# zertovitch/zip-ada

Hardware: NVIDIA B200
Metric: bzip2_encode_MBps_900k (higher is better)
Workload: dtype u8

## Files before the change

zip-ada_b200/csrc/b2_api.cu:

```cuda
#include "b2_common.cuh"
#include "b2_kernels.h"
#include "../../include/b2gpu.h"

#include <algorithm>
#include <atomic>
#include <cmath>
#include <condition_variable>
#include <cstdlib>
#include <cstring>
#include <deque>
#include <chrono>
#include <map>
#include <mutex>
#include <string>
#include <thread>
#include <vector>
#include <unordered_set>

static thread_local std::string g_last_error = "";
void b2_set_error(const char *file, int line, const char *msg) {
  char buf[512];
  snprintf(buf, sizeof buf, "%s:%d: %s", file, line, msg);
  g_last_error = buf;
}
#define B2_FAIL(code, msg) do { b2_set_error(__FILE__, __LINE__, msg); return code; } while (0)
#define B2_TRY(x) do { int rc_ = (x); if (rc_) return rc_; } while (0)

namespace {

template <class T> struct DevBuf {
  T *p = nullptr; size_t cap = 0;
  int ensure(size_t n) {
    if (n <= cap) return 0;
    if (p) cudaFree(p);
    p = nullptr; cap = 0;
    size_t want = n + n / 8 + 256;
    cudaError_t e = cudaMalloc((void **)&p, want * sizeof(T));
    if (e != cudaSuccess) { b2_set_error(__FILE__, __LINE__, cudaGetErrorString(e)); return B2_ERR_ALLOC; }
    cap = want;
    return 0;
  }
  void release() { if (p) cudaFree(p); p = nullptr; cap = 0; }
};

struct ChunkPlan {
  u64 start; u32 len; u32 cap;
  std::vector<u32> tactic_jobs[4];
  u32 n_seg[2];
  int n_tactics;
};

struct Batch {
  u32 c0, c1;
  std::vector<B2Job> jobs;
};

struct Workspace {
  cudaStream_t st = nullptr;
  cudaEvent_t ev[2] = {nullptr, nullptr};
  cudaEvent_t ev_sort[2] = {nullptr, nullptr};
  double sort_ms = 0;
  DevBuf<u32> d_scalars;
  DevBuf<B2Job> d_jobs;
  DevBuf<u8> d_text, d_bwt, d_idx;
  DevBuf<u32> d_m16, d_m256, d_tilemask;
  DevBuf<u64> d_keysA, d_keysB;
  DevBuf<u32> d_valsA, d_valsB, d_rank, d_grp, d_slotA, d_slotB, d_sa, d_tile_cnt;
  DevBuf<B2SortTile> d_tiles, d_mtiles, d_msegs;
  DevBuf<B2SortTileRR> d_tiles_rr;
  DevBuf<B2SortJob> d_sj;
  DevBuf<u32> d_hist, d_digit_base;
  DevBuf<i32> d_tile_head, d_carry;
  DevBuf<u32> d_unsorted;
  DevBuf<u16> d_mtf, d_ghist;
  DevBuf<u8> d_gdist;
  DevBuf<u32> d_rank3, d_rank4;
  DevBuf<u8> d_sel, d_selprev, d_selpos, d_lens;
  DevBuf<u32> d_ehist, d_leaves, d_wl, d_estat, d_selcost;
  DevBuf<u32> d_gpack;
  DevBuf<u16> d_gselcost;
  DevBuf<u32> d_cost, d_low;
  DevBuf<u32> d_bits;
  DevBuf<B2ConcatItem> d_items;
  u32 *h_unsorted = nullptr; size_t h_unsorted_cap = 0;
  std::vector<B2Job> batch_jobs;
  u32 total_groups = 0;
  B2SortStats sort_stats;
  u64 launches = 0, blocks = 0, block_bytes = 0;
  double stage_ms[8] = {0, 0, 0, 0, 0, 0, 0, 0};

  void release() {
    d_scalars.release(); d_jobs.release(); d_text.release(); d_bwt.release(); d_idx.release(); d_m16.release();
    d_m256.release(); d_tilemask.release(); d_keysA.release(); d_keysB.release(); d_valsA.release(); d_valsB.release();
    d_rank.release(); d_grp.release(); d_slotA.release(); d_slotB.release(); d_sa.release(); d_tile_cnt.release(); d_tiles.release(); d_tiles_rr.release(); d_mtiles.release(); d_msegs.release(); d_sj.release(); d_hist.release();
    d_digit_base.release(); d_tile_head.release(); d_carry.release(); d_unsorted.release(); d_mtf.release(); d_ghist.release(); d_gdist.release();
    d_rank3.release(); d_rank4.release(); d_sel.release(); d_selprev.release(); d_selpos.release(); d_lens.release();
    d_ehist.release(); d_leaves.release(); d_wl.release(); d_estat.release(); d_selcost.release(); d_gpack.release(); d_gselcost.release(); d_cost.release();
    d_low.release(); d_bits.release(); d_items.release();
    if (h_unsorted) cudaFreeHost(h_unsorted);
    h_unsorted = nullptr; h_unsorted_cap = 0;
    if (ev[0]) cudaEventDestroy(ev[0]);
    if (ev[1]) cudaEventDestroy(ev[1]);
    if (ev_sort[0]) cudaEventDestroy(ev_sort[0]);
    if (ev_sort[1]) cudaEventDestroy(ev_sort[1]);
    ev_sort[0] = ev_sort[1] = nullptr;
    if (st) cudaStreamDestroy(st);
    st = nullptr; ev[0] = ev[1] = nullptr;
  }
};

}

struct ShardCand { u32 arena; u32 blocks; u64 word_off; u64 nbits; u32 fold; u32 kept; };
struct ShardState {
  bool open = false, cut = false, encoded = false;
  const u8 *d_in = nullptr;
  u64 base = 0, n_local = 0, stream_n = 0, own_end = 0, entry = 0, handoff = 0;
  i64 hint = -1;
  std::vector<DevBuf<u32> *> arenas;
  std::vector<ShardCand> cands;
  std::vector<int> n_tactics;
};

struct b2_encoder {
  int level = 9, device = 0;
  ShardState shard;
  b2_progress_fn progress = nullptr;
  void *progress_user = nullptr;
  cudaStream_t st = nullptr;
  cudaStream_t st2 = nullptr;
  cudaEvent_t ev_fork = nullptr, ev_join = nullptr;
  int timing = 0;
  DevBuf<B2CrcTables> d_ct;
  DevBuf<double> d_T;
  DevBuf<u8> d_in;
  DevBuf<u32> d_out;
  DevBuf<B2Chunk> d_chunks;
  DevBuf<u32> d_scalars;
  DevBuf<u32> d_seg, d_nseg;
  DevBuf<B2StreamEnd> d_ends;
  DevBuf<B2PackItem> d_packitems;
  DevBuf<u8> d_packed;
  DevBuf<u32> d_cut_first, d_cut_last, d_cut_tsum;
  DevBuf<u64> d_cut_carry, d_cut_tincl;
  DevBuf<u8> d_cut_gs;
  DevBuf<u16> d_cut_gm;
  DevBuf<B2ZipCrcTables> d_zt;
  DevBuf<B2ZipTile> d_ztiles;
  DevBuf<B2ZipEntry> d_zents;
  DevBuf<B2ZipCopy> d_zcopies;
  DevBuf<u32> d_zpartial, d_zcrc;
  DevBuf<u8> d_vstream, d_vlcol, d_vrle, d_vsel;
  DevBuf<u32> d_vlink, d_vchain, d_vscal;
  DevBuf<u64> d_vcand;
  DevBuf<B2VBlock> d_vblocks;
  std::vector<Workspace *> ws;
  std::vector<B2Chunk> chunks;
  std::vector<u32> nseg;
  std::vector<std::vector<u32>> seg;
  std::vector<b2_chunk_trace> trace;
  b2_stats stats;
  B2SortStats sort_stats;
  bool batch_positions_fixed = false;
  size_t batch_positions = 1536ull << 20;
  size_t first_batch_positions = ~(size_t)0;
  size_t batch_jobs_max = 65535;
  int n_workspaces = 1;
  u64 launches_other = 0;
  cudaEvent_t ev[2] = {nullptr, nullptr};
  cudaEvent_t ev_call[2] = {nullptr, nullptr};
};

namespace {

struct StageTimer {
  cudaStream_t st; cudaEvent_t *ev; double *acc; bool on;
  StageTimer(b2_encoder *e, cudaStream_t st_, cudaEvent_t *ev_, double *acc_) : st(st_), ev(ev_), acc(acc_), on(e->timing >= 2) {
    if (on) cudaEventRecord(ev[0], st);
  }
  ~StageTimer() {
    if (on) {
      cudaEventRecord(ev[1], st);
      cudaEventSynchronize(ev[1]);
      float ms = 0; cudaEventElapsedTime(&ms, ev[0], ev[1]);
      *acc += ms;
    }
  }
};

void balance_window(int level, i64 &lo, i64 &hi) {
  volatile float fcap = (float)(100000 * level);
  volatile float flo = fcap * 1.05f, fhi = fcap * 1.30f;
  lo = -1; hi = -2;
  i64 base = 100000ll * level;
  for (i64 v = base; v <= 2 * base; v++) {
    volatile float f = (float)v;
    if (f >= flo && f <= fhi) { if (lo < 0) lo = v; hi = v; }
  }
}

int ensure_batch_workspace(Workspace *w, size_t T, size_t J) {
  const size_t max_tiles = T / B2_SORT_TILE + J + 8;
  const size_t max_mtiles = T / B2_MTF_TILE + J + 8;
  const size_t GT = T / B2_GROUP_SIZE + 20 * J + 32;
  B2_TRY(w->d_scalars.ensure(16));
  B2_TRY(w->d_jobs.ensure(J));
  B2_TRY(w->d_text.ensure(T + 64)); B2_TRY(w->d_bwt.ensure(T + 64)); B2_TRY(w->d_idx.ensure(T + 64));
  B2_TRY(w->d_m16.ensure((T / 16 + 8 * J + 8) * 8)); B2_TRY(w->d_m256.ensure((T / 256 + 2 * J + 8) * 8));
  B2_TRY(w->d_keysA.ensure(T)); B2_TRY(w->d_keysB.ensure(T));
  B2_TRY(w->d_valsA.ensure(T)); B2_TRY(w->d_valsB.ensure(T));
  B2_TRY(w->d_rank.ensure(T)); B2_TRY(w->d_grp.ensure(T));
  B2_TRY(w->d_slotA.ensure(T)); B2_TRY(w->d_slotB.ensure(T)); B2_TRY(w->d_sa.ensure(T)); B2_TRY(w->d_tile_cnt.ensure(max_tiles));
  B2_TRY(w->d_tiles.ensure(max_tiles)); B2_TRY(w->d_tiles_rr.ensure(max_tiles)); B2_TRY(w->d_mtiles.ensure(max_mtiles));
  B2_TRY(w->d_tilemask.ensure(max_mtiles * 8)); B2_TRY(w->d_msegs.ensure(T / B2_MTF_SEG + J + 8));
  B2_TRY(w->d_sj.ensure(J));
  B2_TRY(w->d_hist.ensure(max_tiles * 256)); B2_TRY(w->d_digit_base.ensure(J * 8 * 256 + 256));
  B2_TRY(w->d_tile_head.ensure(max_tiles)); B2_TRY(w->d_carry.ensure(max_tiles));
  B2_TRY(w->d_unsorted.ensure(J));
  B2_TRY(w->d_mtf.ensure(T + 16 * J + 64)); B2_TRY(w->d_ghist.ensure(T + 16 * J + 64));
  B2_TRY(w->d_rank3.ensure(GT)); B2_TRY(w->d_rank4.ensure(GT)); B2_TRY(w->d_gdist.ensure(GT));
  B2_TRY(w->d_sel.ensure(GT * B2_N_TRIPLES + 64)); B2_TRY(w->d_selprev.ensure(GT * B2_N_TRIPLES + 64));
  B2_TRY(w->d_selpos.ensure(GT));
  B2_TRY(w->d_gpack.ensure(GT * B2_N_TRIPLES + 64)); B2_TRY(w->d_gselcost.ensure(GT * B2_N_TRIPLES + 64));
  B2_TRY(w->d_ehist.ensure(J * B2_N_TRIPLES * B2_MAX_CODERS * 260));
  B2_TRY(w->d_leaves.ensure((J * B2_N_TRIPLES * B2_MAX_CODERS + 64) * 260)); B2_TRY(w->d_wl.ensure(J * B2_N_TRIPLES * (B2_MAX_CODERS + 3) + J / 32 + 512));
  B2_TRY(w->d_estat.ensure(J * B2_N_TRIPLES * 2)); B2_TRY(w->d_selcost.ensure(J * B2_N_TRIPLES));
  B2_TRY(w->d_lens.ensure(J * B2_N_TRIPLES * B2_MAX_CODERS * B2_MAX_ALPHA));
  B2_TRY(w->d_cost.ensure(J * B2_N_TRIPLES)); B2_TRY(w->d_low.ensure(J * B2_N_TRIPLES));
  B2_TRY(w->d_items.ensure(J));
  if (J > w->h_unsorted_cap) {
    if (w->h_unsorted) cudaFreeHost(w->h_unsorted);
    B2_CUDA_CHECK(cudaMallocHost((void **)&w->h_unsorted, (J + 64) * sizeof(u32)));
    w->h_unsorted_cap = J + 64;
  }
  return 0;
}

u64 layout_jobs(std::vector<B2Job> &jobs, int level) {
  u64 pos = 0, mpos = 0;
  for (auto &j : jobs) {
    u64 cap = std::min<u64>((u64)j.raw_len * 5 / 4 + 8, (u64)level * 100000 + 64);
    cap = (cap + 255) & ~255ull;
    j.pos_off = (u32)pos; j.cap = (u32)cap;
    pos += cap;
    j.mtf_off = (u32)mpos;
    mpos += (cap + 2 + 7) & ~7ull;
  }
  return pos;
}

int run_batch(b2_encoder *e, Workspace *w, const u8 *d_in, std::vector<B2Job> &jobs) {
  const u32 J = (u32)jobs.size();
  if (J == 0) return 0;
  const u64 T = layout_jobs(jobs, e->level);
  if (T >= (1ull << 32) - (1ull << 20)) B2_FAIL(B2_ERR_INTERNAL, "batch too large for 32-bit arena offsets (lower B2GPU_BATCH_POSITIONS)");
  B2_TRY(ensure_batch_workspace(w, (size_t)T + 64, J));
  cudaStream_t st = w->st;
  B2_CUDA_CHECK(cudaMemcpyAsync(w->d_jobs.p, jobs.data(), J * sizeof(B2Job), cudaMemcpyHostToDevice, st));
  {
    StageTimer tm(e, st, w->ev, &w->stage_ms[1]);
    B2_TRY(b2k_rle1(st, d_in, w->d_jobs.p, J, w->d_text.p, e->d_ct.p));
    w->launches += 1;
  }
  w->batch_jobs.resize(J);
  B2_CUDA_CHECK(cudaMemcpyAsync(w->batch_jobs.data(), w->d_jobs.p, J * sizeof(B2Job), cudaMemcpyDeviceToHost, st));
  B2_CUDA_CHECK(cudaStreamSynchronize(st));
  u32 gpos = 0, max_g = 1;
  std::vector<u32> ids(J), ns(J);
  std::vector<B2SortTile> mtiles, msegs, msegs_mid, msegs_big;
  for (u32 j = 0; j < J; j++) {
    B2Job &b = w->batch_jobs[j];
    if (b.n > b.cap) B2_FAIL(B2_ERR_INTERNAL, "RLE1 output exceeds its slot");
    u32 gmax = (b.n / B2_GROUP_SIZE + 2 + 15) & ~15u;
    b.grp_off = gpos; gpos += gmax;
    max_g = std::max(max_g, gmax);
    ids[j] = j; ns[j] = b.n;
    b.na = b.n;
    b.tile0 = (u32)mtiles.size();
    for (u32 s = 0; s < b.n; s += B2_MTF_TILE) mtiles.push_back(B2SortTile{j, s});
    for (u32 s = 0; s < b.n; s += B2_MTF_SEG) (b.n_used <= 64 ? msegs : b.n_used <= 128 ? msegs_mid : msegs_big).push_back(B2SortTile{j, s});
    w->block_bytes += b.n;
  }
  w->blocks += J;
  w->total_groups = gpos;
  B2_CUDA_CHECK(cudaMemcpyAsync(w->d_jobs.p, w->batch_jobs.data(), J * sizeof(B2Job), cudaMemcpyHostToDevice, st));
  {
    StageTimer tm(e, st, w->ev, &w->stage_ms[2]);
    B2SortCtx cx;
    cx.keysA = w->d_keysA.p; cx.keysB = w->d_keysB.p; cx.valsA = w->d_valsA.p; cx.valsB = w->d_valsB.p;
    cx.rank = w->d_rank.p; cx.grp = w->d_grp.p; cx.d_tiles = w->d_tiles.p; cx.d_sj = w->d_sj.p;
    cx.slotA = w->d_slotA.p; cx.slotB = w->d_slotB.p; cx.sa_full = w->d_sa.p; cx.d_tile_cnt = w->d_tile_cnt.p;
    cx.d_hist = w->d_hist.p; cx.d_digit_base = w->d_digit_base.p; cx.d_tiles_rr = w->d_tiles_rr.p; cx.d_ticket = w->d_digit_base.p + w->d_digit_base.cap - 256; cx.d_tile_head = w->d_tile_head.p; cx.d_carry = w->d_carry.p;
    cx.d_unsorted = w->d_unsorted.p; cx.h_unsorted = w->h_unsorted;
    cx.max_tiles = w->d_tiles.cap; cx.max_jobs = w->d_sj.cap; cx.timing = e->timing >= 1;
    cx.stats = w->sort_stats;
    {
      u32 max_used = 1;
      for (u32 j = 0; j < J; j++) max_used = std::max(max_used, w->batch_jobs[j].n_used);
      cx.sym_bits = 1;
      while ((1u << cx.sym_bits) < max_used) cx.sym_bits++;
      cx.max_used = max_used;
      cx.h_jobs = w->batch_jobs.data();
    }
    if (e->timing >= 1) cudaEventRecord(w->ev_sort[0], st);
    int rc = b2k_bwt_batch(&cx, st, w->d_jobs.p, ids, ns, w->d_text.p, w->d_bwt.p);
    if (e->timing >= 1) cudaEventRecord(w->ev_sort[1], st);
    w->sort_stats = cx.stats;
    if (rc) return rc;
  }
  {
    StageTimer tm(e, st, w->ev, &w->stage_ms[3]);
    if (!mtiles.empty())
      B2_CUDA_CHECK(cudaMemcpyAsync(w->d_mtiles.p, mtiles.data(), mtiles.size() * sizeof(B2SortTile), cudaMemcpyHostToDevice, st));
    const u32 n_small = (u32)msegs.size(), n_mid = (u32)msegs_mid.size();
    msegs.insert(msegs.end(), msegs_mid.begin(), msegs_mid.end());
    msegs.insert(msegs.end(), msegs_big.begin(), msegs_big.end());
    if (!msegs.empty())
      B2_CUDA_CHECK(cudaMemcpyAsync(w->d_msegs.p, msegs.data(), msegs.size() * sizeof(B2SortTile), cudaMemcpyHostToDevice, st));
    B2_TRY(b2k_mtf(st, w->d_jobs.p, J, w->d_mtiles.p, (u32)mtiles.size(), w->d_msegs.p, n_small, n_mid, (u32)msegs.size(), w->d_bwt.p, w->d_m16.p,
                   w->d_m256.p, w->d_tilemask.p, w->d_idx.p, w->d_mtf.p));
    w->launches += 4;
  }
  B2_CUDA_CHECK(cudaMemcpyAsync(w->batch_jobs.data(), w->d_jobs.p, J * sizeof(B2Job), cudaMemcpyDeviceToHost, st));
  B2_CUDA_CHECK(cudaStreamSynchronize(st));
  max_g = 1;
  u32 max_alpha = 2;
  for (u32 j = 0; j < J; j++) {
    max_g = std::max(max_g, w->batch_jobs[j].n_groups);
    max_alpha = std::max(max_alpha, w->batch_jobs[j].n_used + 2);
  }
  {
    StageTimer tm(e, st, w->ev, &w->stage_ms[4]);
    B2_TRY(b2k_entropy(st, w->d_jobs.p, J, max_g, gpos, w->d_mtf.p, w->d_ghist.p, w->d_gdist.p, w->d_rank3.p, w->d_rank4.p, w->d_sel.p,
                       w->d_selprev.p, w->d_gpack.p, w->d_gselcost.p, w->d_ehist.p, w->d_leaves.p, w->d_wl.p, w->d_lens.p, w->d_estat.p, w->d_selcost.p,
                       w->d_cost.p, w->d_low.p, e->level, max_alpha, w->d_scalars.p + 8, &w->launches));
  }
  {
    StageTimer tm(e, st, w->ev, &w->stage_ms[5]);
    u64 *d_total = (u64 *)(w->d_scalars.p + 2);
    B2_TRY(b2k_bits_layout(st, w->d_jobs.p, J, d_total));
    u64 total_words = 0;
    B2_CUDA_CHECK(cudaMemcpyAsync(&total_words, d_total, sizeof(u64), cudaMemcpyDeviceToHost, st));
    B2_CUDA_CHECK(cudaStreamSynchronize(st));
    B2_TRY(w->d_bits.ensure(total_words + 64));
    B2_CUDA_CHECK(cudaMemsetAsync(w->d_bits.p, 0, (total_words + 8) * sizeof(u32), st));
    B2_TRY(b2k_pack(st, w->d_jobs.p, J, w->d_mtf.p, w->d_sel.p, w->d_lens.p, w->d_selpos.p, w->d_bits.p, e->level, gpos));
    w->launches += 2;
  }
  B2_CUDA_CHECK(cudaMemcpyAsync(w->batch_jobs.data(), w->d_jobs.p, J * sizeof(B2Job), cudaMemcpyDeviceToHost, st));
  B2_CUDA_CHECK(cudaStreamSynchronize(st));
  if (e->timing >= 1) { float ms = 0; if (cudaEventElapsedTime(&ms, w->ev_sort[0], w->ev_sort[1]) == cudaSuccess) w->sort_ms += ms; }
  return 0;
}

inline u32 rotl1(u32 x) { return (x << 1) | (x >> 31); }

int plan_chunk(b2_encoder *e, u32 c, ChunkPlan &P, std::vector<B2Job> &add, size_t first_id, u64 &addpos) {
  const int level = e->level;
  std::vector<std::pair<u32, u32>> slices[4];
  int nt = 1;
  slices[0].push_back({0, P.len});
  if (level == 9) {
    nt = 4;
    u32 size = P.len / 4, stop = 0;
    for (u32 count = 1; count <= 4; count++) {
      u32 start = stop;
      stop = (count == 4) ? P.len : count * size;
      slices[1].push_back({start, stop - start});
    }
    for (int k = 0; k < 2; k++) {
      u32 ns = e->nseg[2 * c + k];
      P.n_seg[k] = ns;
      if (ns == 0) slices[2 + k].push_back({0, 0});
      else if (ns == 1) slices[2 + k].push_back({0, P.len});
      else {
        const std::vector<u32> &cuts = e->seg[2 * c + k];
        u32 index_start = 0;
        for (u32 s = 0; s < ns; s++) { slices[2 + k].push_back({index_start, cuts[s] - index_start}); index_start = cuts[s]; }
      }
    }
  }
  std::map<std::pair<u32, u32>, u32> seen;
  add.clear(); addpos = 0;
  for (int t = 0; t < nt; t++) {
    P.tactic_jobs[t].clear();
    for (auto &sl : slices[t]) {
      auto it = seen.find(sl);
      u32 id;
      if (it == seen.end()) {
        id = (u32)(first_id + add.size());
        seen[sl] = id;
        B2Job j; memset(&j, 0, sizeof j);
        j.raw_off = P.start + sl.first; j.raw_len = sl.second;
        add.push_back(j);
        addpos += std::min<u64>((u64)sl.second * 5 / 4 + 264, (u64)level * 100000 + 320);
      } else id = it->second;
      P.tactic_jobs[t].push_back(id);
    }
  }
  P.n_tactics = nt;
  return 0;
}

struct StreamDesc {
  u64 off, n; i64 hint;
  u64 out_off, out_len;
  u32 chunk0, n_chunks;
};

void reset_workspace_stats(b2_encoder *e) {
  for (auto *w : e->ws) {
    memset(&w->sort_stats, 0, sizeof w->sort_stats);
    w->launches = 0; w->blocks = 0; w->block_bytes = 0; w->sort_ms = 0;
    for (int i = 0; i < 8; i++) w->stage_ms[i] = 0;
  }
}

void merge_workspace_stats(b2_encoder *e) {
  for (auto *w : e->ws) {
    e->sort_stats.scatter_launches += w->sort_stats.scatter_launches;
    e->sort_stats.scatter_elems += w->sort_stats.scatter_elems;
    e->sort_stats.scatter_ms += w->sort_stats.scatter_ms;
    e->sort_stats.rounds += w->sort_stats.rounds;
    e->sort_stats.sorted_elems_round0 += w->sort_stats.sorted_elems_round0;
    e->sort_stats.sorted_elems_later += w->sort_stats.sorted_elems_later;
    e->sort_stats.launches += w->sort_stats.launches;
    e->launches_other += w->launches;
    e->stats.blocks += w->blocks; e->stats.block_bytes += w->block_bytes; e->stats.sort_ms += w->sort_ms;
    for (int i = 1; i < 8; i++) e->stats.stage_ms[i] += w->stage_ms[i];
  }
  e->stats.sort_rounds = e->sort_stats.rounds;
  e->stats.sort_elems_round0 = e->sort_stats.sorted_elems_round0;
  e->stats.sort_elems_later = e->sort_stats.sorted_elems_later;
  e->stats.scatter_launches = e->sort_stats.scatter_launches;
  e->stats.scatter_elems = e->sort_stats.scatter_elems;
  e->stats.scatter_ms = e->sort_stats.scatter_ms;
  e->stats.kernel_launches = e->launches_other + e->sort_stats.launches;
}

int encode_chunks(b2_encoder *e, const u8 *d_in, std::vector<StreamDesc> &streams, std::vector<u32> &chunk_stream, bool followed,
                  ShardState *sh);

int encode_streams(b2_encoder *e, const u8 *d_in, std::vector<StreamDesc> &streams) {
  cudaStream_t st = e->st;
  const int level = e->level;
  B2_CUDA_CHECK(cudaStreamSynchronize(e->st2));
  e->shard.open = e->shard.cut = e->shard.encoded = false;
  e->trace.clear(); e->chunks.clear(); e->nseg.clear(); e->seg.clear();
  i64 win_lo, win_hi;
  balance_window(level, win_lo, win_hi);
  const i64 full_cap = (i64)level * 100000;
  std::vector<u32> chunk_stream;
  bool followed = false;
  {
    StageTimer tm(e, st, e->ev, &e->stats.stage_ms[0]);
    const u64 small_limit = (u64)((win_lo / 2 - 16) * 4 / 5);
    for (size_t si = 0; si < streams.size(); si++) {
      StreamDesc &S = streams[si];
      e->stats.streams++; e->stats.input_bytes += S.n;
      S.chunk0 = (u32)e->chunks.size();
      if (S.n <= small_limit) {
        const i64 rest = S.hint < 0 ? -1 : S.hint;
        const i64 cap = (rest >= win_lo && rest <= win_hi) ? rest / 2 : full_cap;
        e->chunks.push_back(B2Chunk{S.off, (u32)S.n, (u32)cap, 0, 0});
      } else {
        const u32 max_chunks = (u32)(S.n / (40000ull * level) + 16);
        B2_TRY(e->d_chunks.ensure(max_chunks));
        const size_t ct = (size_t)(S.n / 2048 + 2);
        B2_TRY(e->d_cut_first.ensure(ct)); B2_TRY(e->d_cut_last.ensure(ct)); B2_TRY(e->d_cut_tsum.ensure(ct));
        B2_TRY(e->d_cut_carry.ensure(ct)); B2_TRY(e->d_cut_tincl.ensure(ct));
        B2_TRY(e->d_cut_gs.ensure(ct * 128)); B2_TRY(e->d_cut_gm.ensure(ct * 128));
        B2CutWork cw{e->d_cut_first.p, e->d_cut_last.p, e->d_cut_tsum.p, e->d_cut_carry.p, e->d_cut_tincl.p, e->d_cut_gs.p, e->d_cut_gm.p};
        const bool follow = level == 9 && streams.size() == 1 && e->timing < 2;
        if (follow) {
          B2_TRY(e->d_seg.ensure((size_t)max_chunks * 2 * B2_MAX_SEG));
          B2_TRY(e->d_nseg.ensure((size_t)max_chunks * 2));
          B2_CUDA_CHECK(cudaMemsetAsync(e->d_nseg.p, 0xFE, (size_t)max_chunks * 2 * sizeof(u32), st));
        }
        B2_TRY(b2k_cut(st, d_in + S.off, S.n, S.hint, level, win_lo, win_hi, e->d_chunks.p, e->d_scalars.p, max_chunks, &cw,
                       follow ? e->d_scalars.p + 12 : nullptr, follow ? e->ev_fork : nullptr));
        e->launches_other += 5;
        if (follow) {
          B2_CUDA_CHECK(cudaStreamWaitEvent(e->st2, e->ev_fork, 0));
          B2_TRY(b2k_segment(e->st2, d_in + S.off, e->d_chunks.p, max_chunks, e->d_T.p, e->d_seg.p, e->d_nseg.p, e->d_scalars.p + 12));
          B2_CUDA_CHECK(cudaEventRecord(e->ev_join, e->st2));
          e->launches_other += 1;
          followed = true;
        }
        u32 nc = 0;
        B2_CUDA_CHECK(cudaMemcpyAsync(&nc, e->d_scalars.p, sizeof(u32), cudaMemcpyDeviceToHost, st));
        B2_CUDA_CHECK(cudaStreamSynchronize(st));
        if (nc > max_chunks) B2_FAIL(B2_ERR_INTERNAL, "chunk table overflow");
        const size_t base = e->chunks.size();
        e->chunks.resize(base + nc);
        B2_CUDA_CHECK(cudaMemcpyAsync(e->chunks.data() + base, e->d_chunks.p, nc * sizeof(B2Chunk), cudaMemcpyDeviceToHost, st));
        B2_CUDA_CHECK(cudaStreamSynchronize(st));
        for (size_t c = base; c < e->chunks.size(); c++) e->chunks[c].start += S.off;
      }
      S.n_chunks = (u32)e->chunks.size() - S.chunk0;
      for (u32 c = 0; c < S.n_chunks; c++) chunk_stream.push_back((u32)si);
    }
  }
  return encode_chunks(e, d_in, streams, chunk_stream, followed, nullptr);
}

int encode_chunks(b2_encoder *e, const u8 *d_in, std::vector<StreamDesc> &streams, std::vector<u32> &chunk_stream, bool followed,
                  ShardState *sh) {
  cudaStream_t st = e->st;
  const int level = e->level;
  const u32 n_chunks = (u32)e->chunks.size();
  e->stats.chunks += n_chunks;
  e->trace.resize(n_chunks);
  if (sh) { sh->cands.assign((size_t)n_chunks * 4, ShardCand{0, 0, 0, 0, 0, 0}); sh->n_tactics.assign(n_chunks, 0); }
  {
    StageTimer tm(e, st, e->ev, &e->stats.stage_ms[0]);
    if (!followed) {
      B2_TRY(e->d_chunks.ensure(n_chunks));
      B2_CUDA_CHECK(cudaMemcpyAsync(e->d_chunks.p, e->chunks.data(), n_chunks * sizeof(B2Chunk), cudaMemcpyHostToDevice, st));
    }
    if (level == 9) {
      e->nseg.assign((size_t)n_chunks * 2, 0);
      e->seg.assign((size_t)n_chunks * 2, std::vector<u32>());
      if (!followed) {
        B2_TRY(e->d_seg.ensure((size_t)n_chunks * 2 * B2_MAX_SEG));
        B2_TRY(e->d_nseg.ensure((size_t)n_chunks * 2));
        B2_TRY(b2k_segment(st, d_in, e->d_chunks.p, n_chunks, e->d_T.p, e->d_seg.p, e->d_nseg.p, nullptr));
        e->launches_other += 1;
      }
    }
    B2_CUDA_CHECK(cudaStreamSynchronize(st));
  }
  u32 seg_have = 0;
  auto fetch_seg = [&](u32 upto) -> int {
    if (level != 9 || upto <= seg_have) return 0;
    upto = std::min(n_chunks, std::max(upto, seg_have + 64));
    for (u32 tries = 0;; tries++) {
      B2_CUDA_CHECK(cudaMemcpyAsync(e->nseg.data() + 2 * (size_t)seg_have, e->d_nseg.p + 2 * (size_t)seg_have,
                                    2 * (size_t)(upto - seg_have) * sizeof(u32), cudaMemcpyDeviceToHost, st));
      B2_CUDA_CHECK(cudaStreamSynchronize(st));
      bool all = true, gave_up = false;
      for (u32 k = 2 * seg_have; k < 2 * upto; k++) {
        if (e->nseg[k] == B2_SEG_PENDING) { all = false; break; }
        if (e->nseg[k] == B2_SEG_GAVE_UP) gave_up = true;
      }
      if (all && gave_up) {
        B2_CUDA_CHECK(cudaStreamSynchronize(e->st2));
        B2_CUDA_CHECK(cudaMemcpyAsync(e->d_chunks.p, e->chunks.data(), n_chunks * sizeof(B2Chunk), cudaMemcpyHostToDevice, st));
        B2_TRY(b2k_segment(st, d_in, e->d_chunks.p, n_chunks, e->d_T.p, e->d_seg.p, e->d_nseg.p, nullptr));
        e->launches_other += 1;
        followed = false;
        continue;
      }
      if (all) break;
      if (!followed || tries > 2000000u) B2_FAIL(B2_ERR_INTERNAL, "segmentation results missing");
      std::this_thread::sleep_for(std::chrono::microseconds(50));
    }
    for (u32 k = 2 * seg_have; k < 2 * upto; k++) {
      const u32 ns = e->nseg[k];
      if (ns > B2_MAX_SEG) B2_FAIL(B2_ERR_INTERNAL, "segment table overflow");
      if (ns > 1) {
        e->seg[k].resize(ns);
        B2_CUDA_CHECK(cudaMemcpyAsync(e->seg[k].data(), e->d_seg.p + (size_t)k * B2_MAX_SEG, ns * sizeof(u32), cudaMemcpyDeviceToHost, st));
      }
    }
    B2_CUDA_CHECK(cudaStreamSynchronize(st));
    seg_have = upto;
    return 0;
  };
  u64 out_total = 0;
  for (auto &S : streams) {
    S.out_off = out_total;
    out_total += (b2_bound(S.n) + 1024ull * S.n_chunks + 71) & ~7ull;
  }
  if (!sh) {
    B2_TRY(e->d_out.ensure(out_total / 4 + 16));
    B2_CUDA_CHECK(cudaMemsetAsync(e->d_out.p, 0, (out_total / 4 + 8) * sizeof(u32), st));
    B2_CUDA_CHECK(cudaStreamSynchronize(st));
  }
  std::vector<ChunkPlan> plans(n_chunks);
  std::deque<Batch> batches;
  std::mutex bmu;
  std::condition_variable bcv;
  bool planned_all = false;
  std::vector<B2StreamEnd> ends(streams.size());
  for (size_t si = 0; si < streams.size(); si++) { ends[si].out_off = streams[si].out_off; ends[si].end_bit = 32; ends[si].crc = 0; ends[si].pad = 0; }
  u64 out_words_needed = 0;
  const int W = (e->timing >= 2) ? 1 : std::max<int>(1, (int)e->ws.size());
  reset_workspace_stats(e);
  std::atomic<u32> next{0};
  std::mutex mu;
  std::condition_variable cv;
  u32 turn = 0;
  u32 planned_total = 0xFFFFFFFFu;
  int err = 0;
  std::string err_msg;
  auto worker = [&](int wi) {
    cudaSetDevice(e->device);
    Workspace *w = e->ws[wi];
    for (;;) {
      const u32 b = next.fetch_add(1);
      Batch *B = nullptr;
      {
        std::unique_lock<std::mutex> lk(bmu);
        bcv.wait(lk, [&] { return b < batches.size() || planned_all; });
        if (b < batches.size()) B = &batches[b];
      }
      if (!B) break;
      int rc = 0;
      {
        std::lock_guard<std::mutex> lk(mu);
        if (err) rc = err;
      }
      if (!rc) rc = run_batch(e, w, d_in, B->jobs);
      std::unique_lock<std::mutex> lk(mu);
      cv.wait(lk, [&] { return turn == b; });
      if (!rc && !err && sh) {
        std::vector<B2ConcatItem> items;
        u64 cursor = 0;
        for (u32 c = B->c0; c < B->c1; c++) {
          ChunkPlan &P = plans[c];
          u64 bits[4] = {0, 0, 0, 0};
          for (int t = 0; t < P.n_tactics; t++) for (u32 id : P.tactic_jobs[t]) bits[t] += w->batch_jobs[id].nbits;
          u32 keep = 0;
          for (u32 phase = 0; phase < 8; phase++) {
            int best = 0;
            for (int t = 0; t < P.n_tactics; t++) if (((phase + bits[t]) >> 3) < ((phase + bits[best]) >> 3)) best = t;
            keep |= 1u << best;
          }
          sh->n_tactics[c] = P.n_tactics;
          b2_chunk_trace tr; memset(&tr, 0, sizeof tr);
          tr.start = sh->base + P.start; tr.len = P.len; tr.dyn_capacity = P.cap; tr.n_seg1 = P.n_seg[0]; tr.n_seg2 = P.n_seg[1];
          tr.winner = -1;
          for (int t = 0; t < P.n_tactics; t++) {
            tr.bits[t] = bits[t];
            ShardCand &cd = sh->cands[(size_t)c * 4 + t];
            cd.arena = b; cd.nbits = bits[t]; cd.kept = (keep >> t) & 1u; cd.blocks = (u32)P.tactic_jobs[t].size(); cd.fold = 0;
            for (u32 id : P.tactic_jobs[t]) cd.fold = rotl1(cd.fold) ^ w->batch_jobs[id].crc;
            if (!cd.kept) continue;
            cursor = (cursor + 63) & ~63ull;
            cd.word_off = cursor >> 5;
            for (u32 id : P.tactic_jobs[t]) {
              const B2Job &jb = w->batch_jobs[id];
              items.push_back(B2ConcatItem{jb.bits_off, jb.nbits, cursor});
              cursor += jb.nbits;
            }
          }
          e->trace[c] = tr;
        }
        while (sh->arenas.size() <= b) sh->arenas.push_back(new DevBuf<u32>());
        DevBuf<u32> *ar = sh->arenas[b];
        rc = ar->ensure((cursor >> 5) + 8);
        if (!rc && cudaMemsetAsync(ar->p, 0, ((cursor >> 5) + 8) * sizeof(u32), w->st) != cudaSuccess) rc = B2_ERR_CUDA;
        if (!rc) rc = w->d_items.ensure(items.size() + 1);
        if (!rc && !items.empty() && cudaMemcpyAsync(w->d_items.p, items.data(), items.size() * sizeof(B2ConcatItem), cudaMemcpyHostToDevice, w->st) != cudaSuccess) rc = B2_ERR_CUDA;
        for (size_t i0 = 0; !rc && i0 < items.size(); i0 += 65535) {
          rc = b2k_concat(w->st, w->d_items.p + i0, (u32)std::min<size_t>(65535, items.size() - i0), w->d_bits.p, ar->p);
          w->launches += 1;
        }
        if (!rc && cudaStreamSynchronize(w->st) != cudaSuccess) { rc = B2_ERR_CUDA; b2_set_error(__FILE__, __LINE__, cudaGetErrorString(cudaGetLastError())); }
      } else if (!rc && !err) {
        std::vector<B2ConcatItem> items;
        for (u32 c = B->c0; c < B->c1; c++) {
          ChunkPlan &P = plans[c];
          B2StreamEnd &E = ends[chunk_stream[c]];
          b2_chunk_trace tr; memset(&tr, 0, sizeof tr);
          tr.start = P.start - streams[chunk_stream[c]].off; tr.len = P.len; tr.dyn_capacity = P.cap;
          tr.n_seg1 = P.n_seg[0]; tr.n_seg2 = P.n_seg[1];
          int best = 0;
          const u32 in_bits = (u32)(E.end_bit & 7);
          for (int t = 0; t < P.n_tactics; t++) {
            u64 bits = 0;
            for (u32 id : P.tactic_jobs[t]) bits += w->batch_jobs[id].nbits;
            tr.bits[t] = bits;
            tr.bytes[t] = (in_bits + bits) >> 3;
          }
          for (int t = 0; t < P.n_tactics; t++) if (tr.bytes[t] < tr.bytes[best]) best = t;
          tr.winner = best;
          for (u32 id : P.tactic_jobs[best]) {
            const B2Job &jb = w->batch_jobs[id];
            items.push_back(B2ConcatItem{jb.bits_off, jb.nbits, E.out_off * 8 + E.end_bit});
            E.end_bit += jb.nbits;
            E.crc = rotl1(E.crc) ^ jb.crc;
          }
          e->trace[c] = tr;
          const StreamDesc &S = streams[chunk_stream[c]];
          const u64 region = (b2_bound(S.n) + 1024ull * S.n_chunks + 71) & ~7ull;
          if ((E.end_bit + 128) / 8 > region) { rc = B2_ERR_INTERNAL; b2_set_error(__FILE__, __LINE__, "output bound exceeded"); break; }
        }
        if (!rc) {
          StageTimer tm(e, w->st, w->ev, &w->stage_ms[6]);
          rc = w->d_items.ensure(items.size());
          if (!rc && cudaMemcpyAsync(w->d_items.p, items.data(), items.size() * sizeof(B2ConcatItem), cudaMemcpyHostToDevice, w->st) != cudaSuccess) rc = B2_ERR_CUDA;
          for (size_t i0 = 0; !rc && i0 < items.size(); i0 += 65535)
            rc = b2k_concat(w->st, w->d_items.p + i0, (u32)std::min<size_t>(65535, items.size() - i0), w->d_bits.p, e->d_out.p);
          if (!rc && cudaStreamSynchronize(w->st) != cudaSuccess) { rc = B2_ERR_CUDA; b2_set_error(__FILE__, __LINE__, cudaGetErrorString(cudaGetLastError())); }
          w->launches += 1;
        }
      }
      if (rc && !err) { err = rc; err_msg = g_last_error; }
      turn = b + 1;
      lk.unlock();
      cv.notify_all();
    }
  };
  size_t batch_limit = e->batch_positions;
  if (!e->batch_positions_fixed && W == 1) {
    u64 total_len = 0;
    for (u32 c = 0; c < n_chunks; c++) total_len += e->chunks[c].len;
    const u64 est = (u64)((double)total_len * 2.8) + (u64)n_chunks * 4096;
    size_t free_b = 0, total_b = 0;
    if (est > batch_limit && cudaMemGetInfo(&free_b, &total_b) == cudaSuccess) {
      const size_t have = e->ws[0]->d_keysA.cap;
      const size_t margin = (size_t)12 << 30;
      size_t can = have + (free_b > margin ? (size_t)((double)(free_b - margin) / 52.0) : 0);
      can = std::min<size_t>(can, 4200000000ull);
      if (est <= can) batch_limit = can;
    }
  }
  std::vector<std::thread> th;
  for (int i = 0; i < W; i++) th.emplace_back(worker, i);
  int plan_rc = 0;
  std::string plan_msg;
  {
    u32 published = 0;
    auto publish = [&](Batch &&bt) {
      { std::lock_guard<std::mutex> lk(bmu); batches.push_back(std::move(bt)); }
      bcv.notify_all();
      published++;
    };
    Batch cur; cur.c0 = 0;
    u64 positions = 0;
    std::vector<B2Job> add;
    for (u32 c = 0; c < n_chunks && !plan_rc; c++) {
      ChunkPlan &P = plans[c];
      P.start = e->chunks[c].start; P.len = e->chunks[c].len; P.cap = e->chunks[c].cap;
      P.n_seg[0] = P.n_seg[1] = 0;
      u64 addpos = 0;
      if ((plan_rc = fetch_seg(c + 1))) break;
      if ((plan_rc = plan_chunk(e, c, P, add, cur.jobs.size(), addpos))) break;
      const size_t limit = (followed && published == 0) ? std::min(e->first_batch_positions, batch_limit) : batch_limit;
      if (!cur.jobs.empty() && (positions + addpos > limit || cur.jobs.size() + add.size() > e->batch_jobs_max)) {
        cur.c1 = c;
        publish(std::move(cur));
        cur = Batch(); cur.c0 = c; positions = 0;
        if ((plan_rc = plan_chunk(e, c, P, add, 0, addpos))) break;
      }
      cur.jobs.insert(cur.jobs.end(), add.begin(), add.end());
      positions += addpos;
    }
    if (!plan_rc && n_chunks) { cur.c1 = n_chunks; publish(std::move(cur)); }
    if (plan_rc) {
      plan_msg = g_last_error;
      std::lock_guard<std::mutex> lk(mu);
      if (!err) { err = plan_rc; err_msg = plan_msg; }
    }
    size_t nb_total = 0;
    { std::lock_guard<std::mutex> lk(bmu); planned_all = true; nb_total = batches.size(); }
    bcv.notify_all();
    { std::lock_guard<std::mutex> lk(mu); planned_total = (u32)nb_total; }
    cv.notify_all();
  }
  if (e->progress) {
    u64 total_bytes = 0;
    for (u32 c = 0; c < n_chunks; c++) total_bytes += e->chunks[c].len;
    std::unique_lock<std::mutex> lk(mu);
    u32 seen = 0;
    for (;;) {
      cv.wait(lk, [&] { return turn > seen || err || (planned_total != 0xFFFFFFFFu && turn >= planned_total); });
      if (turn > seen) {
        seen = turn;
        u64 done_bytes = 0;
        { std::lock_guard<std::mutex> lb(bmu); for (u32 b = 0; b < seen && b < batches.size(); b++) for (u32 c = batches[b].c0; c < batches[b].c1; c++) done_bytes += e->chunks[c].len; }
        lk.unlock();
        const int stop = e->progress(e->progress_user, done_bytes, total_bytes);
        lk.lock();
        if (stop && !err) { err = B2_ERR_ABORTED; err_msg = "aborted by the progress callback (User_abort)"; }
      }
      if (err || (planned_total != 0xFFFFFFFFu && turn >= planned_total)) break;
    }
  }
  for (auto &t : th) t.join();
  if (followed) B2_CUDA_CHECK(cudaStreamSynchronize(e->st2));
  (void)out_words_needed;
  if (err) { g_last_error = err_msg; return err; }
  if (!sh) {
    B2_TRY(e->d_ends.ensure(ends.size()));
    B2_CUDA_CHECK(cudaMemcpyAsync(e->d_ends.p, ends.data(), ends.size() * sizeof(B2StreamEnd), cudaMemcpyHostToDevice, st));
    B2_TRY(b2k_stream_ends(st, e->d_ends.p, (u32)ends.size(), level, e->d_out.p));
    e->launches_other += 1;
    B2_CUDA_CHECK(cudaStreamSynchronize(st));
    for (size_t si = 0; si < streams.size(); si++) streams[si].out_len = (ends[si].end_bit + 80 + 7) >> 3;
  }
  merge_workspace_stats(e);
  return 0;
}

int encode_device(b2_encoder *e, const u8 *d_in, u64 n, i64 size_hint, u64 *out_len) {
  std::vector<StreamDesc> streams(1);
  streams[0] = StreamDesc{0, n, size_hint, 0, 0, 0, 0};
  B2_TRY(encode_streams(e, d_in, streams));
  *out_len = streams[0].out_len;
  return 0;
}

}

namespace {
int zip_crc_device(b2_encoder *e, const u8 *d_in, u32 n_entries, const u64 *offs, const u64 *sizes) {
  if (!e->d_zt.p) {
    B2ZipCrcTables *zt = new B2ZipCrcTables();
    b2k_make_zipcrc_tables(zt);
    int rc = e->d_zt.ensure(1);
    if (!rc && cudaMemcpy(e->d_zt.p, zt, sizeof(B2ZipCrcTables), cudaMemcpyHostToDevice) != cudaSuccess) rc = B2_ERR_CUDA;
    delete zt;
    if (rc) B2_FAIL(rc, "zip crc tables");
  }
  std::vector<B2ZipTile> tiles;
  std::vector<B2ZipEntry> ents(n_entries);
  for (u32 i = 0; i < n_entries; i++) {
    const u64 nt = (sizes[i] + B2_ZIP_TILE - 1) / B2_ZIP_TILE;
    ents[i] = B2ZipEntry{sizes[i], (u32)tiles.size(), (u32)nt};
    for (u64 k = 0; k < nt; k++) tiles.push_back(B2ZipTile{offs[i], offs[i] + sizes[i] - (nt - 1 - k) * (u64)B2_ZIP_TILE});
  }
  if (tiles.size() >= (1ull << 31)) B2_FAIL(B2_ERR_ARGUMENT, "too much input for one archive call");
  B2_TRY(e->d_ztiles.ensure(tiles.size() + 1));
  B2_TRY(e->d_zents.ensure(n_entries + 1));
  B2_TRY(e->d_zpartial.ensure(tiles.size() + 1));
  B2_TRY(e->d_zcrc.ensure(n_entries + 1));
  if (!tiles.empty()) B2_CUDA_CHECK(cudaMemcpyAsync(e->d_ztiles.p, tiles.data(), tiles.size() * sizeof(B2ZipTile), cudaMemcpyHostToDevice, e->st));
  if (n_entries) B2_CUDA_CHECK(cudaMemcpyAsync(e->d_zents.p, ents.data(), n_entries * sizeof(B2ZipEntry), cudaMemcpyHostToDevice, e->st));
  B2_TRY(b2k_zipcrc(e->st, d_in, e->d_ztiles.p, (u32)tiles.size(), e->d_zents.p, n_entries, e->d_zt.p, e->d_zpartial.p, e->d_zcrc.p));
  e->launches_other += 2;
  B2_CUDA_CHECK(cudaStreamSynchronize(e->st));
  return 0;
}

struct ByteSink {
  std::vector<u8> b;
  void u16le(u32 v) { b.push_back((u8)v); b.push_back((u8)(v >> 8)); }
  void u32le(u64 v) { for (int k = 0; k < 4; k++) b.push_back((u8)(v >> (8 * k))); }
  void u64le(u64 v) { for (int k = 0; k < 8; k++) b.push_back((u8)(v >> (8 * k))); }
  void sig(u8 c1, u8 c2) { b.push_back(0x50); b.push_back(0x4B); b.push_back(c1); b.push_back(c2); }
  void str(const std::string &s) { b.insert(b.end(), s.begin(), s.end()); }
};
struct HeaderSpan { u64 dst; std::vector<u8> bytes; };
}


extern "C" {

const char *b2_last_error(void) { return g_last_error.c_str(); }

uint64_t b2_bound(uint64_t n) { return n + n / 50 + 4096; }

int b2_create(int level, int device, b2_encoder **out) {
  if (!out) B2_FAIL(B2_ERR_ARGUMENT, "out is NULL");
  *out = nullptr;
  if (level != 1 && level != 4 && level != 9) B2_FAIL(B2_ERR_ARGUMENT, "level must be 1, 4 or 9");
  int ndev = 0;
  cudaError_t ce = cudaGetDeviceCount(&ndev);
  if (ce != cudaSuccess || ndev == 0) B2_FAIL(B2_ERR_CUDA, "no CUDA device available (b2gpu has no CPU fallback)");
  if (device < 0 || device >= ndev) B2_FAIL(B2_ERR_ARGUMENT, "bad device index");
  B2_CUDA_CHECK(cudaSetDevice(device));
  b2_encoder *e = new b2_encoder();
  e->level = level; e->device = device;
  memset(&e->stats, 0, sizeof e->stats);
  memset(&e->sort_stats, 0, sizeof e->sort_stats);
  if (const char *s = getenv("B2GPU_BATCH_POSITIONS")) { long long v = atoll(s); if (v >= (1 << 20)) { e->batch_positions = (size_t)std::min<long long>(v, 3ll << 30); e->batch_positions_fixed = true; } }
  if (const char *s = getenv("B2GPU_FIRST_BATCH_POSITIONS")) { long long v = atoll(s); if (v >= (1 << 20)) e->first_batch_positions = (size_t)v; }
  if (const char *s = getenv("B2GPU_BATCH_JOBS")) { long long v = atoll(s); if (v >= 8) e->batch_jobs_max = (size_t)std::min<long long>(v, 65535); }
  if (const char *s = getenv("B2GPU_PIPELINE")) { int v = atoi(s); if (v >= 1 && v <= 8) e->n_workspaces = v; }
  auto init = [&]() -> int {
    B2_CUDA_CHECK(cudaStreamCreateWithFlags(&e->st, cudaStreamNonBlocking));
    B2_CUDA_CHECK(cudaStreamCreateWithFlags(&e->st2, cudaStreamNonBlocking));
    B2_CUDA_CHECK(cudaEventCreateWithFlags(&e->ev_fork, cudaEventDisableTiming));
    B2_CUDA_CHECK(cudaEventCreateWithFlags(&e->ev_join, cudaEventDisableTiming));
    B2_CUDA_CHECK(cudaEventCreate(&e->ev[0])); B2_CUDA_CHECK(cudaEventCreate(&e->ev[1]));
    B2_CUDA_CHECK(cudaEventCreate(&e->ev_call[0])); B2_CUDA_CHECK(cudaEventCreate(&e->ev_call[1]));
    for (int i = 0; i < e->n_workspaces; i++) {
      Workspace *w = new Workspace();
      e->ws.push_back(w);
      B2_CUDA_CHECK(cudaStreamCreateWithFlags(&w->st, cudaStreamNonBlocking));
      B2_CUDA_CHECK(cudaEventCreate(&w->ev[0])); B2_CUDA_CHECK(cudaEventCreate(&w->ev[1]));
      B2_CUDA_CHECK(cudaEventCreate(&w->ev_sort[0])); B2_CUDA_CHECK(cudaEventCreate(&w->ev_sort[1]));
    }
    {
      std::vector<B2CrcTables> ct(1);
      b2k_make_crc_tables(ct.data());
      B2_TRY(e->d_ct.ensure(1));
      B2_CUDA_CHECK(cudaMemcpy(e->d_ct.p, ct.data(), sizeof(B2CrcTables), cudaMemcpyHostToDevice));
    }
    std::vector<double> T(16002, 0.0);
    const double inv = 1.0 / 16000.0;
    for (int c = 1; c <= 16001; c++) { double p = (double)c * inv; T[c] = -(p * std::log(p)); }
    B2_TRY(e->d_T.ensure(T.size()));
    B2_CUDA_CHECK(cudaMemcpy(e->d_T.p, T.data(), T.size() * sizeof(double), cudaMemcpyHostToDevice));
    B2_TRY(e->d_scalars.ensure(16));
    return 0;
  };
  const int rc = init();
  if (rc) { const std::string msg = g_last_error; b2_destroy(e); g_last_error = msg; return rc; }
  *out = e;
  return 0;
}

void b2_destroy(b2_encoder *e) {
  if (!e) return;
  cudaSetDevice(e->device);
  if (e->st) cudaStreamSynchronize(e->st);
  for (auto *w : e->ws) { if (w->st) cudaStreamSynchronize(w->st); w->release(); delete w; }
  e->ws.clear();
  e->d_ct.release(); e->d_T.release(); e->d_in.release(); e->d_out.release(); e->d_chunks.release();
  e->d_scalars.release(); e->d_seg.release(); e->d_nseg.release(); e->d_ends.release(); e->d_packitems.release(); e->d_packed.release(); e->d_cut_first.release(); e->d_cut_last.release();
  e->d_cut_tsum.release(); e->d_cut_carry.release(); e->d_cut_tincl.release(); e->d_cut_gs.release(); e->d_cut_gm.release();
  e->d_vstream.release(); e->d_vlcol.release(); e->d_vrle.release(); e->d_vsel.release(); e->d_vlink.release(); e->d_vchain.release();
  e->d_vscal.release(); e->d_vcand.release(); e->d_vblocks.release();
  e->d_zt.release(); e->d_ztiles.release(); e->d_zents.release(); e->d_zcopies.release(); e->d_zpartial.release(); e->d_zcrc.release();
  if (e->ev[0]) cudaEventDestroy(e->ev[0]);
  if (e->ev[1]) cudaEventDestroy(e->ev[1]);
  if (e->ev_call[0]) cudaEventDestroy(e->ev_call[0]);
  if (e->ev_call[1]) cudaEventDestroy(e->ev_call[1]);
  if (e->st2) { cudaStreamSynchronize(e->st2); cudaStreamDestroy(e->st2); }
  if (e->ev_fork) cudaEventDestroy(e->ev_fork);
  if (e->ev_join) cudaEventDestroy(e->ev_join);
  if (e->st) cudaStreamDestroy(e->st);
  delete e;
}

int b2_encode_stream_device(b2_encoder *e, const uint8_t *d_in, uint64_t n, int64_t size_hint,
                            uint8_t *d_out, uint64_t out_cap, uint64_t *out_len) {
  if (!e || !out_len || (n && !d_in)) B2_FAIL(B2_ERR_ARGUMENT, "bad argument");
  B2_CUDA_CHECK(cudaSetDevice(e->device));
  u64 len = 0;
  if (e->timing) cudaEventRecord(e->ev_call[0], e->st);
  B2_TRY(encode_device(e, d_in, n, size_hint, &len));
  *out_len = len;
  if (len > out_cap) B2_FAIL(B2_ERR_OUTPUT_TOO_SMALL, "output buffer too small");
  if (d_out) B2_CUDA_CHECK(cudaMemcpyAsync(d_out, e->d_out.p, len, cudaMemcpyDeviceToDevice, e->st));
  if (e->timing) cudaEventRecord(e->ev_call[1], e->st);
  B2_CUDA_CHECK(cudaStreamSynchronize(e->st));
  if (e->timing) { float ms = 0; cudaEventElapsedTime(&ms, e->ev_call[0], e->ev_call[1]); e->stats.call_ms += ms; }
  return 0;
}

int b2_encode_stream(b2_encoder *e, const uint8_t *in, uint64_t n, int64_t size_hint,
                     uint8_t *out, uint64_t out_cap, uint64_t *out_len) {
  if (!e || !out_len || (n && !in)) B2_FAIL(B2_ERR_ARGUMENT, "bad argument");
  B2_CUDA_CHECK(cudaSetDevice(e->device));
  B2_TRY(e->d_in.ensure(n + 256));
  if (e->timing) cudaEventRecord(e->ev_call[0], e->st);
  {
    StageTimer tm(e, e->st, e->ev, &e->stats.stage_ms[7]);
    if (n) B2_CUDA_CHECK(cudaMemcpyAsync(e->d_in.p, in, n, cudaMemcpyHostToDevice, e->st));
    B2_CUDA_CHECK(cudaMemsetAsync(e->d_in.p + n, 0, 128, e->st));
  }
  u64 len = 0;
  B2_TRY(encode_device(e, e->d_in.p, n, size_hint, &len));
  *out_len = len;
  if (len > out_cap) B2_FAIL(B2_ERR_OUTPUT_TOO_SMALL, "output buffer too small");
  {
    StageTimer tm(e, e->st, e->ev, &e->stats.stage_ms[7]);
    if (out) B2_CUDA_CHECK(cudaMemcpyAsync(out, e->d_out.p, len, cudaMemcpyDeviceToHost, e->st));
    if (e->timing) cudaEventRecord(e->ev_call[1], e->st);
    B2_CUDA_CHECK(cudaStreamSynchronize(e->st));
  }
  if (e->timing) { float ms = 0; cudaEventElapsedTime(&ms, e->ev_call[0], e->ev_call[1]); e->stats.call_ms += ms; }
  return 0;
}

int b2_encode_batch(b2_encoder *e, uint32_t n_entries, const uint8_t *in, const uint64_t *in_offsets,
                    const uint64_t *sizes, const int64_t *size_hints, uint8_t *out, uint64_t out_cap,
                    uint64_t *out_offsets, uint64_t *out_lens) {
  if (!e || (n_entries && (!in_offsets || !sizes || !out_offsets || !out_lens))) B2_FAIL(B2_ERR_ARGUMENT, "bad argument");
  B2_CUDA_CHECK(cudaSetDevice(e->device));
  u64 total_in = 0;
  for (u32 i = 0; i < n_entries; i++) total_in = std::max<u64>(total_in, in_offsets[i] + sizes[i]);
  if (total_in && !in) B2_FAIL(B2_ERR_ARGUMENT, "bad argument");
  B2_TRY(e->d_in.ensure(total_in + 256));
  if (e->timing) cudaEventRecord(e->ev_call[0], e->st);
  if (total_in) B2_CUDA_CHECK(cudaMemcpyAsync(e->d_in.p, in, total_in, cudaMemcpyHostToDevice, e->st));
  B2_CUDA_CHECK(cudaMemsetAsync(e->d_in.p + total_in, 0, 128, e->st));
  std::vector<StreamDesc> streams(n_entries);
  for (u32 i = 0; i < n_entries; i++) streams[i] = StreamDesc{in_offsets[i], sizes[i], size_hints ? size_hints[i] : -1, 0, 0, 0, 0};
  B2_TRY(encode_streams(e, e->d_in.p, streams));
  std::vector<B2PackItem> items(n_entries);
  u64 pos = 0;
  for (u32 i = 0; i < n_entries; i++) {
    items[i] = B2PackItem{streams[i].out_off, pos, streams[i].out_len};
    out_offsets[i] = pos; out_lens[i] = streams[i].out_len;
    pos += (streams[i].out_len + 7) & ~7ull;
  }
  if (pos > out_cap) B2_FAIL(B2_ERR_OUTPUT_TOO_SMALL, "output buffer too small");
  if (n_entries) {
    B2_TRY(e->d_packitems.ensure(n_entries));
    B2_TRY(e->d_packed.ensure(pos + 64));
    B2_CUDA_CHECK(cudaMemcpyAsync(e->d_packitems.p, items.data(), n_entries * sizeof(B2PackItem), cudaMemcpyHostToDevice, e->st));
    B2_TRY(b2k_pack_streams(e->st, e->d_packitems.p, n_entries, (const u8 *)e->d_out.p, e->d_packed.p));
    if (out && pos) B2_CUDA_CHECK(cudaMemcpyAsync(out, e->d_packed.p, pos, cudaMemcpyDeviceToHost, e->st));
  }
  if (e->timing) cudaEventRecord(e->ev_call[1], e->st);
  B2_CUDA_CHECK(cudaStreamSynchronize(e->st));
  if (e->timing) { float ms = 0; cudaEventElapsedTime(&ms, e->ev_call[0], e->ev_call[1]); e->stats.call_ms += ms; }
  return 0;
}

uint64_t b2_shard_margin(int level) { return 10ull * 100000ull * (u64)level + 4096; }

int b2_shard_plan(uint64_t n, int n_shards, int level, int stagger_permille, uint64_t *bounds) {
  if (!bounds || n_shards < 1) return B2_ERR_ARGUMENT;
  (void)level;
  if (stagger_permille < 0) {
    stagger_permille = 12;
    if (const char *sv = getenv("B2GPU_SHARD_STAGGER")) { int v = atoi(sv); if (v >= 0 && v < 500) stagger_permille = v; }
  }
  const double q = 1.0 - stagger_permille / 1000.0;
  double tot = 0, w = 1;
  for (int r = 0; r < n_shards; r++) { tot += w; w *= q; }
  double acc = 0; w = 1;
  bounds[0] = 0;
  for (int r = 0; r < n_shards; r++) {
    acc += w; w *= q;
    u64 b = (u64)((double)n * (acc / tot));
    b &= ~4095ull;
    if (b < bounds[r]) b = bounds[r];
    bounds[r + 1] = r + 1 == n_shards ? n : std::min<u64>(b, n);
  }
  return 0;
}

int b2_shard_resolve(const b2_shard_link *links, int n_shards, uint64_t *bit_offsets, uint32_t *crcs) {
  if (!links || !bit_offsets || !crcs || n_shards < 1) return B2_ERR_ARGUMENT;
  bit_offsets[0] = 32; crcs[0] = 0;
  for (int r = 0; r < n_shards; r++) {
    const u32 ph = (u32)(bit_offsets[r] & 7);
    bit_offsets[r + 1] = bit_offsets[r] + links[r].total_bits[ph];
    const u32 k = links[r].crc_rot[ph] & 31u, c = crcs[r];
    crcs[r + 1] = (k ? ((c << k) | (c >> (32 - k))) : c) ^ links[r].crc_fold[ph];
  }
  return 0;
}

int b2_shard_open(b2_encoder *e, const uint8_t *in, int in_is_device, uint64_t base, uint64_t n_local,
                  uint64_t stream_size, int64_t size_hint, uint64_t own_end) {
  if (!e || (n_local && !in) || base + n_local > stream_size || own_end > stream_size || own_end < base) B2_FAIL(B2_ERR_ARGUMENT, "bad argument");
  B2_CUDA_CHECK(cudaSetDevice(e->device));
  B2_CUDA_CHECK(cudaStreamSynchronize(e->st2));
  ShardState &sh = e->shard;
  sh.open = sh.cut = sh.encoded = false;
  sh.base = base; sh.n_local = n_local; sh.stream_n = stream_size; sh.hint = size_hint; sh.own_end = own_end;
  if (e->timing) cudaEventRecord(e->ev_call[0], e->st);
  if (in_is_device) sh.d_in = in;
  else {
    B2_TRY(e->d_in.ensure(n_local + 256));
    if (n_local) B2_CUDA_CHECK(cudaMemcpyAsync(e->d_in.p, in, n_local, cudaMemcpyHostToDevice, e->st));
    B2_CUDA_CHECK(cudaMemsetAsync(e->d_in.p + n_local, 0, 128, e->st));
    sh.d_in = e->d_in.p;
  }
  const size_t ct = (size_t)(n_local / 2048 + 2);
  B2_TRY(e->d_cut_first.ensure(ct)); B2_TRY(e->d_cut_last.ensure(ct)); B2_TRY(e->d_cut_tsum.ensure(ct));
  B2_TRY(e->d_cut_carry.ensure(ct)); B2_TRY(e->d_cut_tincl.ensure(ct));
        B2_TRY(e->d_cut_gs.ensure(ct * 128)); B2_TRY(e->d_cut_gm.ensure(ct * 128));
  B2CutWork cw{e->d_cut_first.p, e->d_cut_last.p, e->d_cut_tsum.p, e->d_cut_carry.p, e->d_cut_tincl.p, e->d_cut_gs.p, e->d_cut_gm.p};
  B2_TRY(b2k_cut_scans(e->st, sh.d_in, n_local, &cw));
  e->launches_other += 4;
  sh.open = true;
  return 0;
}

int b2_shard_cut(b2_encoder *e, uint64_t entry, uint64_t *handoff) {
  if (!e || !handoff) B2_FAIL(B2_ERR_ARGUMENT, "bad argument");
  ShardState &sh = e->shard;
  if (!sh.open) B2_FAIL(B2_ERR_ARGUMENT, "b2_shard_cut without b2_shard_open");
  if (entry < sh.base || entry > sh.base + sh.n_local) B2_FAIL(B2_ERR_ARGUMENT, "entry outside the shard's bytes");
  B2_CUDA_CHECK(cudaSetDevice(e->device));
  cudaStream_t st = e->st;
  const int level = e->level;
  e->trace.clear(); e->chunks.clear(); e->nseg.clear(); e->seg.clear();
  i64 win_lo, win_hi;
  balance_window(level, win_lo, win_hi);
  const u64 own = sh.own_end > entry ? sh.own_end - entry : 0;
  const u32 max_chunks = (u32)(own / (40000ull * level) + 16);
  B2_TRY(e->d_chunks.ensure(max_chunks));
  B2CutWork cw{e->d_cut_first.p, e->d_cut_last.p, e->d_cut_tsum.p, e->d_cut_carry.p, e->d_cut_tincl.p, e->d_cut_gs.p, e->d_cut_gm.p};
  const bool follow = level == 9 && e->timing < 2;
  if (level == 9) {
    B2_TRY(e->d_seg.ensure((size_t)max_chunks * 2 * B2_MAX_SEG));
    B2_TRY(e->d_nseg.ensure((size_t)max_chunks * 2));
    B2_CUDA_CHECK(cudaMemsetAsync(e->d_nseg.p, 0xFE, (size_t)max_chunks * 2 * sizeof(u32), st));
  }
  const bool last = sh.own_end >= sh.stream_n;
  const u64 stop = last ? sh.n_local : sh.own_end - sh.base;
  B2_TRY(b2k_cut_chain(st, sh.d_in, sh.n_local, sh.hint, level, win_lo, win_hi, e->d_chunks.p, e->d_scalars.p, max_chunks, &cw,
                       follow ? e->d_scalars.p + 12 : nullptr, follow ? e->ev_fork : nullptr, sh.base, entry - sh.base, stop));
  e->launches_other += 1;
  if (follow) {
    B2_CUDA_CHECK(cudaStreamWaitEvent(e->st2, e->ev_fork, 0));
    B2_TRY(b2k_segment(e->st2, sh.d_in, e->d_chunks.p, max_chunks, e->d_T.p, e->d_seg.p, e->d_nseg.p, e->d_scalars.p + 12));
    B2_CUDA_CHECK(cudaEventRecord(e->ev_join, e->st2));
    e->launches_other += 1;
  }
  u32 sc[4] = {0, 0, 0, 0};
  B2_CUDA_CHECK(cudaMemcpyAsync(sc, e->d_scalars.p, sizeof sc, cudaMemcpyDeviceToHost, st));
  B2_CUDA_CHECK(cudaStreamSynchronize(st));
  const u32 nc = sc[0];
  if (nc > max_chunks) B2_FAIL(B2_ERR_INTERNAL, "chunk table overflow");
  e->chunks.resize(nc);
  if (nc) B2_CUDA_CHECK(cudaMemcpy(e->chunks.data(), e->d_chunks.p, nc * sizeof(B2Chunk), cudaMemcpyDeviceToHost));
  sh.entry = entry;
  sh.handoff = sh.base + ((u64)sc[2] | ((u64)sc[3] << 32));
  *handoff = sh.handoff;
  sh.cut = true;
  return 0;
}

int b2_shard_encode(b2_encoder *e, b2_shard_link *link) {
  if (!e || !link) B2_FAIL(B2_ERR_ARGUMENT, "bad argument");
  ShardState &sh = e->shard;
  if (!sh.cut) B2_FAIL(B2_ERR_ARGUMENT, "b2_shard_encode without b2_shard_cut");
  B2_CUDA_CHECK(cudaSetDevice(e->device));
  const u32 nc = (u32)e->chunks.size();
  std::vector<StreamDesc> streams(1);
  streams[0] = StreamDesc{0, sh.n_local, sh.hint, 0, 0, 0, nc};
  e->stats.streams++; e->stats.input_bytes += sh.handoff - sh.entry;
  std::vector<u32> chunk_stream(nc, 0u);
  const bool followed = e->level == 9 && e->timing < 2;
  B2_TRY(encode_chunks(e, sh.d_in, streams, chunk_stream, followed, &sh));
  for (u32 phase0 = 0; phase0 < 8; phase0++) {
    u64 total = 0; u32 rot = 0, fold = 0, ph = phase0;
    for (u32 c = 0; c < nc; c++) {
      const ShardCand *cd = &sh.cands[(size_t)c * 4];
      int best = 0;
      for (int t = 0; t < sh.n_tactics[c]; t++) if (((ph + cd[t].nbits) >> 3) < ((ph + cd[best].nbits) >> 3)) best = t;
      total += cd[best].nbits; ph = (u32)((ph + cd[best].nbits) & 7);
      const u32 k = cd[best].blocks & 31u;
      fold = (k ? ((fold << k) | (fold >> (32 - k))) : fold) ^ cd[best].fold;
      rot = (rot + cd[best].blocks) & 31u;
    }
    link->total_bits[phase0] = total; link->crc_rot[phase0] = rot; link->crc_fold[phase0] = fold;
  }
  sh.encoded = true;
  return 0;
}

int b2_shard_finish(b2_encoder *e, uint64_t bit_offset, uint32_t crc_in, uint8_t *out, int out_is_device, uint64_t out_cap,
                    uint64_t *out_byte_offset, uint64_t *out_len, uint8_t *first_byte, uint8_t *last_byte) {
  if (!e || !out_len || !out_byte_offset) B2_FAIL(B2_ERR_ARGUMENT, "bad argument");
  ShardState &sh = e->shard;
  if (!sh.encoded) B2_FAIL(B2_ERR_ARGUMENT, "b2_shard_finish without b2_shard_encode");
  B2_CUDA_CHECK(cudaSetDevice(e->device));
  cudaStream_t st = e->st;
  const bool first = sh.base == 0 && sh.entry == 0, last = sh.own_end >= sh.stream_n;
  if (first && bit_offset != 32) B2_FAIL(B2_ERR_ARGUMENT, "the first shard starts behind the 32-bit stream header");
  const u64 byte0 = first ? 0 : bit_offset >> 3;
  const u64 lbit0 = bit_offset - 8 * byte0;
  const u32 nc = (u32)e->chunks.size();
  std::vector<std::vector<B2ConcatItem>> items(sh.arenas.size());
  u64 lbit = lbit0;
  u32 crc = crc_in;
  for (u32 c = 0; c < nc; c++) {
    const ShardCand *cd = &sh.cands[(size_t)c * 4];
    const u32 in_bits = (u32)(lbit & 7);
    int best = 0;
    b2_chunk_trace &tr = e->trace[c];
    for (int t = 0; t < sh.n_tactics[c]; t++) tr.bytes[t] = (in_bits + cd[t].nbits) >> 3;
    for (int t = 0; t < sh.n_tactics[c]; t++) if (tr.bytes[t] < tr.bytes[best]) best = t;
    tr.winner = best;
    if (!cd[best].kept) B2_FAIL(B2_ERR_INTERNAL, "the winning candidate was not kept");
    if (cd[best].arena >= items.size()) B2_FAIL(B2_ERR_INTERNAL, "candidate arena missing");
    items[cd[best].arena].push_back(B2ConcatItem{cd[best].word_off, cd[best].nbits, lbit});
    lbit += cd[best].nbits;
    const u32 k = cd[best].blocks & 31u;
    crc = (k ? ((crc << k) | (crc >> (32 - k))) : crc) ^ cd[best].fold;
  }
  const u64 end_bit = lbit + (last ? 80 : 0);
  const u64 len = (end_bit + 7) >> 3;
  *out_len = len; *out_byte_offset = byte0;
  if (len > out_cap) B2_FAIL(B2_ERR_OUTPUT_TOO_SMALL, "output buffer too small");
  B2_TRY(e->d_out.ensure(len / 4 + 16));
  B2_CUDA_CHECK(cudaMemsetAsync(e->d_out.p, 0, (len / 4 + 8) * sizeof(u32), st));
  Workspace *w = e->ws[0];
  for (size_t a = 0; a < items.size(); a++) {
    if (items[a].empty()) continue;
    B2_TRY(w->d_items.ensure(items[a].size()));
    B2_CUDA_CHECK(cudaMemcpyAsync(w->d_items.p, items[a].data(), items[a].size() * sizeof(B2ConcatItem), cudaMemcpyHostToDevice, st));
    for (size_t i0 = 0; i0 < items[a].size(); i0 += 65535) {
      B2_TRY(b2k_concat(st, w->d_items.p + i0, (u32)std::min<size_t>(65535, items[a].size() - i0), sh.arenas[a]->p, e->d_out.p));
      e->launches_other += 1;
    }
    B2_CUDA_CHECK(cudaStreamSynchronize(st));
  }
  if (first || last) {
    B2StreamEnd E{0, lbit, crc, (first ? 0u : 1u) | (last ? 0u : 2u)};
    B2_TRY(e->d_ends.ensure(1));
    B2_CUDA_CHECK(cudaMemcpyAsync(e->d_ends.p, &E, sizeof E, cudaMemcpyHostToDevice, st));
    B2_TRY(b2k_stream_ends(st, e->d_ends.p, 1, e->level, e->d_out.p));
    e->launches_other += 1;
  }
  if (out && len) B2_CUDA_CHECK(cudaMemcpyAsync(out, e->d_out.p, len, out_is_device ? cudaMemcpyDeviceToDevice : cudaMemcpyDeviceToHost, st));
  u8 fb[2] = {0, 0};
  if (len) {
    B2_CUDA_CHECK(cudaMemcpyAsync(&fb[0], e->d_out.p, 1, cudaMemcpyDeviceToHost, st));
    B2_CUDA_CHECK(cudaMemcpyAsync(&fb[1], (const u8 *)e->d_out.p + (len - 1), 1, cudaMemcpyDeviceToHost, st));
  }
  if (e->timing) cudaEventRecord(e->ev_call[1], st);
  B2_CUDA_CHECK(cudaStreamSynchronize(st));
  if (first_byte) *first_byte = fb[0];
  if (last_byte) *last_byte = fb[1];
  if (e->timing) { float ms = 0; cudaEventElapsedTime(&ms, e->ev_call[0], e->ev_call[1]); e->stats.call_ms += ms; }
  sh.encoded = false; sh.cut = false; sh.open = false;
  return 0;
}

int b2_encode_stream_multi(b2_encoder **encs, int n_encs, const uint8_t *in, uint64_t n, int64_t size_hint,
                           uint8_t *out, uint64_t out_cap, uint64_t *out_len) {
  if (!encs || n_encs < 1 || !out_len || (n && !in)) B2_FAIL(B2_ERR_ARGUMENT, "bad argument");
  for (int i = 0; i < n_encs; i++) if (!encs[i] || encs[i]->level != encs[0]->level) B2_FAIL(B2_ERR_ARGUMENT, "handles must share the block size");
  const int level = encs[0]->level;
  u64 min_share = 64ull << 20;
  if (const char *sv = getenv("B2GPU_SHARD_MIN_BYTES")) { long long v = atoll(sv); if (v >= 65536) min_share = (u64)v; }
  const int ns = (int)std::max<u64>(1, std::min<u64>((u64)n_encs, n / min_share));
  if (ns == 1) return b2_encode_stream(encs[0], in, n, size_hint, out, out_cap, out_len);
  std::vector<u64> bounds(ns + 1);
  B2_TRY(b2_shard_plan(n, ns, level, -1, bounds.data()));
  const u64 margin = b2_shard_margin(level);
  std::vector<b2_shard_link> links(ns);
  std::vector<u64> entry(ns + 1, 0), bit_off(ns + 1, 0), piece_off(ns, 0), piece_len(ns, 0);
  std::vector<u32> crcs(ns + 1, 0);
  std::vector<u8> fb(ns, 0), lb(ns, 0);
  std::vector<int> rcs(ns, 0);
  std::vector<std::string> msgs(ns);
  std::mutex mu;
  std::condition_variable cv;
  int cut_done = 0, enc_done = 0;
  bool failed = false, resolved = false;
  auto run = [&](int r) {
    b2_encoder *e = encs[r];
    int rc = 0;
    auto fail = [&](int code) {
      rc = code; msgs[r] = g_last_error;
      { std::lock_guard<std::mutex> lk(mu); failed = true; }
      cv.notify_all();
    };
    const u64 lo = bounds[r], hi = std::min<u64>(n, bounds[r + 1] + (r + 1 < ns ? margin : 0));
    if ((rc = b2_shard_open(e, in + lo, 0, lo, hi - lo, n, size_hint, bounds[r + 1]))) { fail(rc); rcs[r] = rc; return; }
    {
      std::unique_lock<std::mutex> lk(mu);
      cv.wait(lk, [&] { return cut_done == r || failed; });
      if (failed) { rcs[r] = B2_ERR_INTERNAL; return; }
    }
    u64 ho = 0;
    if ((rc = b2_shard_cut(e, entry[r], &ho))) { fail(rc); rcs[r] = rc; return; }
    { std::lock_guard<std::mutex> lk(mu); entry[r + 1] = ho; cut_done = r + 1; }
    cv.notify_all();
    if ((rc = b2_shard_encode(e, &links[r]))) { fail(rc); rcs[r] = rc; return; }
    {
      std::unique_lock<std::mutex> lk(mu);
      enc_done++;
      if (enc_done == ns) {
        b2_shard_resolve(links.data(), ns, bit_off.data(), crcs.data());
        resolved = true;
        cv.notify_all();
      }
      cv.wait(lk, [&] { return resolved || failed; });
      if (failed) { rcs[r] = B2_ERR_INTERNAL; return; }
    }
    const u64 total = (bit_off[ns] + 80 + 7) >> 3;
    if (total > out_cap) { b2_set_error(__FILE__, __LINE__, "output buffer too small"); fail(B2_ERR_OUTPUT_TOO_SMALL); rcs[r] = B2_ERR_OUTPUT_TOO_SMALL; return; }
    const u64 b0 = r == 0 ? 0 : bit_off[r] >> 3;
    if ((rc = b2_shard_finish(e, bit_off[r], crcs[r], out + b0, 0, out_cap - b0, &piece_off[r], &piece_len[r], &fb[r], &lb[r]))) { fail(rc); rcs[r] = rc; return; }
  };
  std::vector<std::thread> th;
  for (int r = 0; r < ns; r++) th.emplace_back(run, r);
  for (auto &t : th) t.join();
  for (int r = 0; r < ns; r++) if (rcs[r] && !msgs[r].empty()) { g_last_error = msgs[r]; return rcs[r]; }
  for (int r = 0; r < ns; r++) if (rcs[r]) return rcs[r];
  std::map<u64, u8> edge;
  for (int r = 0; r < ns; r++) {
    if (!piece_len[r]) continue;
    edge[piece_off[r]] |= fb[r];
    edge[piece_off[r] + piece_len[r] - 1] |= lb[r];
  }
  for (auto &kv : edge) out[kv.first] = kv.second;
  *out_len = (bit_off[ns] + 80 + 7) >> 3;
  return 0;
}

int b2_verify_stream(b2_encoder *e, const uint8_t *stream, int stream_is_device, uint64_t n, const uint8_t *expect,
                     int expect_is_device, uint64_t expect_n, b2_verify_result *res) {
  if (!e || !res || (n && !stream)) B2_FAIL(B2_ERR_ARGUMENT, "bad argument");
  memset(res, 0, sizeof *res);
  res->first_bad_block = -1; res->mismatch_at = ~0ull;
  B2_CUDA_CHECK(cudaSetDevice(e->device));
  cudaStream_t st = e->st;
  if (n < 14) { res->first_bad_status = 1; return 0; }
  B2_TRY(e->d_vstream.ensure(n + 128));
  B2_CUDA_CHECK(cudaEventRecord(e->ev[0], st));
  B2_CUDA_CHECK(cudaMemcpyAsync(e->d_vstream.p, stream, n, stream_is_device ? cudaMemcpyDeviceToDevice : cudaMemcpyHostToDevice, st));
  B2_CUDA_CHECK(cudaMemsetAsync(e->d_vstream.p + n, 0, 128, st));
  u8 head[4];
  B2_CUDA_CHECK(cudaMemcpyAsync(head, e->d_vstream.p, 4, cudaMemcpyDeviceToHost, st));
  B2_CUDA_CHECK(cudaStreamSynchronize(st));
  if (head[0] != 'B' || head[1] != 'Z' || head[2] != 'h' || head[3] < '1' || head[3] > '9') { res->first_bad_status = 1; return 0; }
  const u32 level = head[3] - '0';
  res->level = level;
  const u32 max_n = level * 100000u;
  const u32 cap = (u32)std::min<u64>(n / 32 + 4096, 1u << 26);
  B2_TRY(e->d_vcand.ensure(cap));
  B2_TRY(e->d_vscal.ensure(8));
  B2_CUDA_CHECK(cudaMemsetAsync(e->d_vscal.p, 0, 8 * sizeof(u32), st));
  B2_TRY(b2k_verify_find(st, e->d_vstream.p, n, e->d_vcand.p, e->d_vscal.p, cap));
  u32 n_cand = 0;
  B2_CUDA_CHECK(cudaMemcpyAsync(&n_cand, e->d_vscal.p, sizeof(u32), cudaMemcpyDeviceToHost, st));
  B2_CUDA_CHECK(cudaStreamSynchronize(st));
  if (n_cand > cap) B2_FAIL(B2_ERR_INTERNAL, "too many block-magic candidates");
  std::vector<u64> cand(n_cand);
  if (n_cand) B2_CUDA_CHECK(cudaMemcpy(cand.data(), e->d_vcand.p, n_cand * sizeof(u64), cudaMemcpyDeviceToHost));
  std::sort(cand.begin(), cand.end());
  res->candidates = n_cand;
  const u8 *d_expect = nullptr;
  if (expect) {
    if (expect_is_device) d_expect = expect;
    else {
      B2_TRY(e->d_in.ensure(expect_n + 256));
      if (expect_n) B2_CUDA_CHECK(cudaMemcpyAsync(e->d_in.p, expect, expect_n, cudaMemcpyHostToDevice, st));
      d_expect = e->d_in.p;
    }
    const unsigned long long none = ~0ull;
    B2_CUDA_CHECK(cudaMemcpyAsync(e->d_vscal.p + 2, &none, sizeof none, cudaMemcpyHostToDevice, st));
  }
  size_t wave = 2048;
  if (const char *sv = getenv("B2GPU_VERIFY_WAVE")) { long v = atol(sv); if (v >= 1) wave = (size_t)v; }
  u64 cur = 32, raw_total = 0;
  u32 combined = 0;
  bool done = false, failed = false;
  u64 n_chain = 0;
  std::vector<B2VBlock> blk;
  std::vector<u32> chain;
  for (size_t c0 = 0; c0 < cand.size() && !done && !failed;) {
    while (c0 < cand.size() && (cand[c0] >> 1) < cur) c0++;
    if (c0 >= cand.size()) break;
    const size_t c1 = std::min(cand.size(), c0 + wave);
    const u32 nb = (u32)(c1 - c0);
    blk.assign(nb, B2VBlock{});
    for (u32 k = 0; k < nb; k++) { blk[k].start_bit = cand[c0 + k] >> 1; blk[k].status = (cand[c0 + k] & 1) ? 0xFFu : 0u; }
    B2_TRY(e->d_vblocks.ensure(nb));
    B2_TRY(e->d_vlink.ensure((size_t)nb * (max_n + 32)));
    B2_TRY(e->d_vlcol.ensure((size_t)nb * (max_n + 32)));
    B2_TRY(e->d_vrle.ensure((size_t)nb * (max_n + 32)));
    B2_TRY(e->d_vsel.ensure((size_t)nb * 18016));
    B2_CUDA_CHECK(cudaMemcpyAsync(e->d_vblocks.p, blk.data(), nb * sizeof(B2VBlock), cudaMemcpyHostToDevice, st));
    B2_TRY(b2k_verify_decode(st, e->d_vstream.p, n, e->d_vblocks.p, nb, max_n, e->d_vlink.p, e->d_vlcol.p, e->d_vrle.p, e->d_vsel.p,
                             e->d_ct.p->byte_tab));
    e->launches_other += 1;
    B2_CUDA_CHECK(cudaMemcpyAsync(blk.data(), e->d_vblocks.p, nb * sizeof(B2VBlock), cudaMemcpyDeviceToHost, st));
    B2_CUDA_CHECK(cudaStreamSynchronize(st));
    chain.clear();
    size_t k = 0;
    while (k < nb) {
      if (blk[k].start_bit < cur) { k++; continue; }
      if (blk[k].start_bit > cur) { failed = true; res->first_bad_block = (int32_t)n_chain; res->first_bad_status = 20; break; }
      if (cand[c0 + k] & 1) {
        u8 f[12];
        B2_CUDA_CHECK(cudaMemcpy(f, e->d_vstream.p + ((cur + 48) >> 3), 8, cudaMemcpyDeviceToHost));
        const u32 sh = (u32)((cur + 48) & 7);
        u64 w = 0;
        for (int q = 0; q < 8; q++) w = (w << 8) | f[q];
        res->stored_stream_crc = (u32)((w << sh) >> 32);
        res->computed_stream_crc = combined;
        const u64 end_bytes = (cur + 80 + 7) >> 3;
        done = true;
        if (end_bytes != n) { failed = true; res->first_bad_status = 21; }
        break;
      }
      const B2VBlock &b = blk[k];
      if (b.status != 0 || b.computed_crc != b.stored_crc) {
        failed = true; res->first_bad_block = (int32_t)n_chain; res->first_bad_status = b.status ? b.status : 30;
        break;
      }
      blk[k].raw_off = raw_total;
      raw_total += b.raw_len;
      combined = rotl1(combined) ^ b.stored_crc;
      cur = b.end_bit;
      chain.push_back((u32)k);
      n_chain++;
      k++;
    }
    if (d_expect && !chain.empty()) {
      B2_TRY(e->d_vchain.ensure(chain.size()));
      B2_CUDA_CHECK(cudaMemcpyAsync(e->d_vblocks.p, blk.data(), nb * sizeof(B2VBlock), cudaMemcpyHostToDevice, st));
      B2_CUDA_CHECK(cudaMemcpyAsync(e->d_vchain.p, chain.data(), chain.size() * sizeof(u32), cudaMemcpyHostToDevice, st));
      B2_TRY(b2k_verify_compare(st, e->d_vblocks.p, e->d_vchain.p, (u32)chain.size(), max_n, e->d_vrle.p, d_expect, expect_n,
                                (unsigned long long *)(e->d_vscal.p + 2)));
      e->launches_other += 1;
      B2_CUDA_CHECK(cudaStreamSynchronize(st));
    }
    c0 = c1;
  }
  if (!done && !failed) { failed = true; res->first_bad_block = (int32_t)n_chain; res->first_bad_status = 22; }
  res->blocks = n_chain;
  res->decoded_bytes = raw_total;
  if (d_expect) {
    unsigned long long bad = ~0ull;
    B2_CUDA_CHECK(cudaMemcpy(&bad, e->d_vscal.p + 2, sizeof bad, cudaMemcpyDeviceToHost));
    res->mismatch_at = bad;
    if (bad == ~0ull && !failed && raw_total != expect_n) res->mismatch_at = std::min<u64>(raw_total, expect_n);
  }
  B2_CUDA_CHECK(cudaEventRecord(e->ev[1], st));
  B2_CUDA_CHECK(cudaStreamSynchronize(st));
  { float ms = 0; cudaEventElapsedTime(&ms, e->ev[0], e->ev[1]); res->ms = ms; }
  res->ok = (!failed && done && res->stored_stream_crc == res->computed_stream_crc && (!d_expect || res->mismatch_at == ~0ull)) ? 1 : 0;
  return 0;
}

uint64_t b2_zip_bound(uint32_t n_entries, uint64_t total_name_bytes, uint64_t total_input_bytes) {
  return (u64)n_entries * (30 + 20 + 46 + 28) + 2 * total_name_bytes + total_input_bytes + 56 + 20 + 22;
}

int b2_zip_crc32(b2_encoder *e, const uint8_t *in, uint64_t n, uint32_t *crc) {
  if (!e || !crc || (n && !in)) B2_FAIL(B2_ERR_ARGUMENT, "bad argument");
  B2_CUDA_CHECK(cudaSetDevice(e->device));
  B2_TRY(e->d_in.ensure(n + 256));
  if (n) B2_CUDA_CHECK(cudaMemcpyAsync(e->d_in.p, in, n, cudaMemcpyHostToDevice, e->st));
  const u64 off = 0;
  B2_TRY(zip_crc_device(e, e->d_in.p, 1, &off, &n));
  B2_CUDA_CHECK(cudaMemcpy(crc, e->d_zcrc.p, sizeof(u32), cudaMemcpyDeviceToHost));
  return 0;
}

int b2_zip_create(b2_encoder *e, uint32_t n_entries, const uint8_t *in, const uint64_t *in_offsets, const uint64_t *sizes,
                  const char *names, const uint32_t *name_offsets, const uint32_t *dos_times, const uint32_t *flags,
                  int duplicates, uint8_t *out, uint64_t out_cap, uint64_t *out_len, b2_zip_entry_info *info) {
  if (!e || !out_len || (n_entries && (!in_offsets || !sizes || !names || !name_offsets))) B2_FAIL(B2_ERR_ARGUMENT, "bad argument");
  B2_CUDA_CHECK(cudaSetDevice(e->device));
  std::vector<std::string> nm(n_entries);
  {
    std::unordered_set<std::string> seen;
    for (u32 i = 0; i < n_entries; i++) {
      if (name_offsets[i + 1] < name_offsets[i] || name_offsets[i + 1] - name_offsets[i] > 65535u) B2_FAIL(B2_ERR_ARGUMENT, "bad entry name length");
      nm[i].assign(names + name_offsets[i], names + name_offsets[i + 1]);
      for (char &c : nm[i]) if (c == '\\') c = '/';
      if (duplicates == B2_ZIP_ERROR_ON_DUPLICATE && !seen.insert(nm[i]).second) {
        g_last_error = "Duplicate_name: Entry name = " + nm[i];
        return B2_ERR_DUPLICATE_NAME;
      }
    }
  }
  u64 total_in = 0;
  for (u32 i = 0; i < n_entries; i++) total_in = std::max<u64>(total_in, in_offsets[i] + sizes[i]);
  if (total_in && !in) B2_FAIL(B2_ERR_ARGUMENT, "bad argument");
  B2_TRY(e->d_in.ensure(total_in + 256));
  if (e->timing) cudaEventRecord(e->ev_call[0], e->st);
  if (total_in) B2_CUDA_CHECK(cudaMemcpyAsync(e->d_in.p, in, total_in, cudaMemcpyHostToDevice, e->st));
  B2_CUDA_CHECK(cudaMemsetAsync(e->d_in.p + total_in, 0, 128, e->st));
  B2_TRY(zip_crc_device(e, e->d_in.p, n_entries, in_offsets, sizes));
  std::vector<u32> crc(n_entries);
  if (n_entries) B2_CUDA_CHECK(cudaMemcpyAsync(crc.data(), e->d_zcrc.p, n_entries * sizeof(u32), cudaMemcpyDeviceToHost, e->st));
  std::vector<StreamDesc> streams(n_entries);
  for (u32 i = 0; i < n_entries; i++) streams[i] = StreamDesc{in_offsets[i], sizes[i], (i64)sizes[i], 0, 0, 0, 0};
  B2_TRY(encode_streams(e, e->d_in.p, streams));
  B2_CUDA_CHECK(cudaStreamSynchronize(e->st));

  const u64 four_gib = 1ull << 32, max_size = 0x1FFFFFFFFFFFFFFFull;
  const u64 margin = 22 + 56 + 20 + 65536 + 10;
  bool zip64 = false;
  auto check_size = [&](u64 value) -> int {
    if (!zip64 && value >= four_gib - margin) {
      zip64 = true;
      if (value >= max_size - margin) return 1;
    }
    return 0;
  };
  std::vector<HeaderSpan> spans;
  std::vector<B2ZipCopy> copies;
  struct Cat { u64 usize, csize, offset; u32 crc, time, ext_attr; u16 flag, method; };
  std::vector<Cat> cat(n_entries);
  u64 pos = 0;
  for (u32 i = 0; i < n_entries; i++) {
    Cat &c = cat[i];
    const u32 fl = flags ? flags[i] : 0;
    c.flag = (fl & B2_ZIP_UNICODE_NAME) ? 0x0800 : 0;
    c.ext_attr = (fl & B2_ZIP_READ_ONLY) ? 1u : 0u;
    c.time = dos_times ? dos_times[i] : 16789u * 65536u;
    c.usize = sizes[i];
    c.crc = crc[i];
    if (check_size(sizes[i])) B2_FAIL(B2_ERR_ARGUMENT, "Zip_Capacity_Exceeded: archive too large");
    c.offset = pos;
    const bool ext = sizes[i] >= 0xFFFFFFFFull || c.offset >= 0xFFFFFFFFull;
    const bool stored = streams[i].out_len >= sizes[i];
    c.method = stored ? 0 : 12;
    c.csize = stored ? sizes[i] : streams[i].out_len;
    ByteSink h;
    h.sig(3, 4);
    h.u16le(10); h.u16le(c.flag); h.u16le(c.method); h.u32le(c.time); h.u32le(c.crc);
    if (ext) { h.u32le(0xFFFFFFFFu); h.u32le(0xFFFFFFFFu); } else { h.u32le(c.csize); h.u32le(c.usize); }
    h.u16le((u32)nm[i].size()); h.u16le(ext ? 20 : 0);
    h.str(nm[i]);
    if (ext) { h.u16le(1); h.u16le(16); h.u64le(c.usize); h.u64le(c.csize); }
    const u64 payload = pos + h.b.size();
    spans.push_back(HeaderSpan{pos, std::move(h.b)});
    const u64 src = stored ? in_offsets[i] : streams[i].out_off;
    for (u64 o = 0; o < c.csize; o += 65536) copies.push_back(B2ZipCopy{src + o, payload + o, (u32)std::min<u64>(65536, c.csize - o), stored ? 1u : 0u});
    pos = payload + c.csize;
    if (info) { info[i].crc32 = c.crc; info[i].zip_type = c.method; info[i].reserved = 0; info[i].compressed_size = c.csize; info[i].local_header_offset = c.offset; }
  }
  {
    ByteSink d;
    const u64 cd_offset = pos;
    u64 cd_size = 0;
    if (!zip64 && n_entries >= 65535u) zip64 = true;
    for (u32 i = 0; i < n_entries; i++) {
      const Cat &c = cat[i];
      const bool ext = c.csize >= 0xFFFFFFFFull || c.usize >= 0xFFFFFFFFull || c.offset >= 0xFFFFFFFFull;
      if (ext) zip64 = true;
      d.sig(1, 2);
      d.u16le(23); d.u16le(10); d.u16le(c.flag); d.u16le(c.method); d.u32le(c.time); d.u32le(c.crc);
      d.u32le(ext ? 0xFFFFFFFFull : c.csize); d.u32le(ext ? 0xFFFFFFFFull : c.usize);
      d.u16le((u32)nm[i].size()); d.u16le(ext ? 28 : 0);
      d.u16le(0); d.u16le(0); d.u16le(0); d.u32le(c.ext_attr);
      d.u32le(ext ? 0xFFFFFFFFull : c.offset);
      d.str(nm[i]);
      if (ext) { d.u16le(1); d.u16le(24); d.u64le(c.usize); d.u64le(c.csize); d.u64le(c.offset); }
      cd_size += 46 + nm[i].size() + (ext ? 28 : 0);
    }
    if (n_entries) { if (check_size(cd_offset + cd_size + 1)) B2_FAIL(B2_ERR_ARGUMENT, "Zip_Capacity_Exceeded: archive too large"); }
    u64 tot = n_entries, dtot = n_entries, cds = cd_size, cdo = cd_offset;
    if (zip64) {
      d.sig(6, 6);
      d.u64le(44); d.u16le(0x2D); d.u16le(0x2D); d.u32le(0); d.u32le(0); d.u64le(n_entries); d.u64le(n_entries); d.u64le(cd_size); d.u64le(cd_offset);
      d.sig(6, 7);
      d.u32le(0); d.u64le(cd_offset + cd_size); d.u32le(1);
      tot = dtot = 0xFFFF; cds = 0xFFFFFFFFull; cdo = 0xFFFFFFFFull;
    }
    d.sig(5, 6);
    d.u16le(0); d.u16le(0); d.u16le((u32)dtot); d.u16le((u32)tot); d.u32le(cds); d.u32le(cdo); d.u16le(0);
    const u64 n = d.b.size();
    spans.push_back(HeaderSpan{pos, std::move(d.b)});
    pos += n;
  }
  *out_len = pos;
  if (pos > out_cap) B2_FAIL(B2_ERR_OUTPUT_TOO_SMALL, "output buffer too small");
  if (!out) B2_FAIL(B2_ERR_ARGUMENT, "out is NULL");
  if (!copies.empty()) {
    if (copies.size() >= (1ull << 31)) B2_FAIL(B2_ERR_ARGUMENT, "too much output for one archive call");
    B2_TRY(e->d_zcopies.ensure(copies.size()));
    B2_TRY(e->d_packed.ensure(pos + 64));
    B2_CUDA_CHECK(cudaMemcpyAsync(e->d_zcopies.p, copies.data(), copies.size() * sizeof(B2ZipCopy), cudaMemcpyHostToDevice, e->st));
    B2_TRY(b2k_zip_gather(e->st, e->d_zcopies.p, (u32)copies.size(), (const u8 *)e->d_out.p, e->d_in.p, e->d_packed.p));
    e->launches_other += 1;
    const u64 first = copies.front().dst_off, last = copies.back().dst_off + copies.back().len;
    B2_CUDA_CHECK(cudaMemcpyAsync(out + first, e->d_packed.p + first, last - first, cudaMemcpyDeviceToHost, e->st));
  }
  if (e->timing) cudaEventRecord(e->ev_call[1], e->st);
  B2_CUDA_CHECK(cudaStreamSynchronize(e->st));
  for (const HeaderSpan &sp : spans) memcpy(out + sp.dst, sp.bytes.data(), sp.bytes.size());
  if (e->timing) { float ms = 0; cudaEventElapsedTime(&ms, e->ev_call[0], e->ev_call[1]); e->stats.call_ms += ms; }
  return 0;
}

int b2_set_timing(b2_encoder *e, int on) { if (!e) return B2_ERR_ARGUMENT; e->timing = on; return 0; }
int b2_get_stats(b2_encoder *e, b2_stats *out) { if (!e || !out) return B2_ERR_ARGUMENT; *out = e->stats; return 0; }
int b2_reset_stats(b2_encoder *e) {
  if (!e) return B2_ERR_ARGUMENT;
  memset(&e->stats, 0, sizeof e->stats); memset(&e->sort_stats, 0, sizeof e->sort_stats);
  e->launches_other = 0;
  return 0;
}

int b2_set_progress(b2_encoder *e, b2_progress_fn fn, void *user) {
  if (!e) return B2_ERR_ARGUMENT;
  e->progress = fn; e->progress_user = user;
  return 0;
}

int b2_get_trace(b2_encoder *e, b2_chunk_trace *out, uint64_t cap, uint64_t *n) {
  if (!e || !n || (cap && !out)) return B2_ERR_ARGUMENT;
  *n = e->trace.size();
  for (size_t i = 0; i < e->trace.size() && i < cap; i++) out[i] = e->trace[i];
  return 0;
}

int b2_get_segments(b2_encoder *e, uint64_t chunk, int profile, uint32_t *cuts, uint32_t cap, uint32_t *n) {
  if (!e || !n || profile < 0 || profile > 1) return B2_ERR_ARGUMENT;
  const size_t k = chunk * 2 + profile;
  if (k >= e->nseg.size()) { *n = 0; return B2_ERR_ARGUMENT; }
  const u32 ns = e->nseg[k];
  *n = ns;
  if (ns == 1 && cap >= 1) cuts[0] = e->chunks[chunk].len;
  else for (u32 i = 0; i < ns && i < cap; i++) cuts[i] = e->seg[k][i];
  return 0;
}

int b2_dbg_block(b2_encoder *e, const uint8_t *raw, uint32_t len, uint8_t *rle_out, uint8_t *bwt_out,
                 uint16_t *mtf_out, uint8_t *sel_out, uint8_t *lens_out, uint8_t *bits_out, uint64_t bits_cap,
                 b2_block_info *info) {
  if (!e || (len && !raw)) B2_FAIL(B2_ERR_ARGUMENT, "bad argument");
  B2_CUDA_CHECK(cudaSetDevice(e->device));
  Workspace *w = e->ws[0];
  cudaStream_t st = w->st;
  B2_TRY(e->d_in.ensure((size_t)len + 256));
  if (len) B2_CUDA_CHECK(cudaMemcpyAsync(e->d_in.p, raw, len, cudaMemcpyHostToDevice, st));
  B2_CUDA_CHECK(cudaMemsetAsync(e->d_in.p + len, 0, 128, st));
  std::vector<B2Job> jobs(1);
  memset(&jobs[0], 0, sizeof(B2Job));
  jobs[0].raw_off = 0; jobs[0].raw_len = len;
  reset_workspace_stats(e);
  memset(&e->sort_stats, 0, sizeof e->sort_stats);
  e->launches_other = 0;
  B2_TRY(run_batch(e, w, e->d_in.p, jobs));
  merge_workspace_stats(e);
  const B2Job &b = w->batch_jobs[0];
  if (rle_out && b.n) B2_CUDA_CHECK(cudaMemcpyAsync(rle_out, w->d_text.p + b.pos_off, b.n, cudaMemcpyDeviceToHost, st));
  if (bwt_out && b.n) B2_CUDA_CHECK(cudaMemcpyAsync(bwt_out, w->d_bwt.p + b.pos_off, b.n, cudaMemcpyDeviceToHost, st));
  if (mtf_out) B2_CUDA_CHECK(cudaMemcpyAsync(mtf_out, w->d_mtf.p + b.mtf_off, (size_t)b.n_mtf * 2, cudaMemcpyDeviceToHost, st));
  const u32 total_groups = w->total_groups;
  if (sel_out) B2_CUDA_CHECK(cudaMemcpyAsync(sel_out, w->d_sel.p + (size_t)b.best * total_groups + b.grp_off, b.n_groups, cudaMemcpyDeviceToHost, st));
  if (lens_out) B2_CUDA_CHECK(cudaMemcpyAsync(lens_out, w->d_lens.p + (size_t)b.best * (B2_MAX_CODERS * B2_MAX_ALPHA), B2_MAX_CODERS * B2_MAX_ALPHA, cudaMemcpyDeviceToHost, st));
  u64 nbytes = (b.nbits + 7) >> 3;
  if (bits_out) {
    if (nbytes > bits_cap) B2_FAIL(B2_ERR_OUTPUT_TOO_SMALL, "bits_out too small");
    B2_CUDA_CHECK(cudaMemcpyAsync(bits_out, (u8 *)(w->d_bits.p + b.bits_off), nbytes, cudaMemcpyDeviceToHost, st));
  }
  B2_CUDA_CHECK(cudaStreamSynchronize(st));
  if (info) {
    int max_len, sw, ec;
    b2_triple(e->level, (int)b.best, max_len, sw, ec);
    info->n_rle = b.n; info->origin = b.origin; info->crc = b.crc; info->n_mtf = b.n_mtf; info->eob = b.n_used + 1;
    info->n_used = b.n_used; info->n_sel = b.n_groups; info->ec_count = (u32)ec; info->max_len = (u32)max_len;
    info->sample_width = (u32)sw; info->cost = b.best_cost; info->pad = 0; info->bits = b.nbits;
  }
  return 0;
}

}
```

zip-ada_b200/csrc/b2_chunks.cu:

```cuda
#include "b2_common.cuh"
#include "b2_kernels.h"

#define CT_TILE 2048
#define CT_THREADS 128
#define NONE32 0xFFFFFFFFu
#define B2_TRY_K(x) do { int rc_ = (x); if (rc_) return rc_; } while (0)

__device__ __forceinline__ u32 enc_size(u32 len) { return (len < 4 ? len : 4) + (len >= 4 ? 1 : 0); }

__device__ __forceinline__ void load16(const u8 *__restrict__ in, u64 base, u64 n_alloc, u8 *b) {
  if (base + 16 <= n_alloc && ((reinterpret_cast<uintptr_t>(in + base)) & 15u) == 0) {
    const uint4 v = *reinterpret_cast<const uint4 *>(in + base);
    const u32 w[4] = {v.x, v.y, v.z, v.w};
#pragma unroll
    for (int k = 0; k < 16; k++) b[k] = (u8)(w[k >> 2] >> (8 * (k & 3)));
  } else {
#pragma unroll
    for (int k = 0; k < 16; k++) b[k] = (base + k < n_alloc) ? in[base + k] : 0;
  }
}

__global__ void __launch_bounds__(CT_THREADS)
k_cut_a(const u8 *__restrict__ in, u64 n, u32 *__restrict__ firstchg, u32 *__restrict__ lastchg) {
  __shared__ u32 s_first, s_last;
  const u64 t0 = (u64)blockIdx.x * CT_TILE;
  const u32 tid = threadIdx.x;
  if (tid == 0) { s_first = NONE32; s_last = 0; }
  __syncthreads();
  const u64 base = t0 + tid * 16;
  u8 b[16];
  load16(in, base, n, b);
  u8 pv = (base > 0 && base < n) ? in[base - 1] : 0;
  u32 f = NONE32, l = 0;
#pragma unroll
  for (int k = 0; k < 16; k++) {
    const u64 p = base + k;
    if (p < n && (p == 0 || b[k] != pv)) { const u32 o = tid * 16 + k; if (f == NONE32) f = o; l = o + 1; }
    pv = b[k];
  }
#pragma unroll
  for (int o = 16; o; o >>= 1) {
    f = min(f, __shfl_xor_sync(0xffffffffu, f, o));
    l = max(l, __shfl_xor_sync(0xffffffffu, l, o));
  }
  if (lane_id() == 0) { if (f != NONE32) atomicMin(&s_first, f); if (l) atomicMax(&s_last, l); }
  __syncthreads();
  if (tid == 0) { firstchg[blockIdx.x] = s_first; lastchg[blockIdx.x] = s_last; }
}

__global__ void __launch_bounds__(1024)
k_cut_s1(const u32 *__restrict__ lastchg, u64 ntiles, u64 *__restrict__ carry_r) {
  __shared__ u64 sm[1024];
  const u32 tid = threadIdx.x;
  const u64 per = (ntiles + 1023) / 1024;
  const u64 a = tid * per, e = min(ntiles, a + per);
  u64 loc = 0;
  for (u64 t = a; t < e; t++) { u32 l = lastchg[t]; if (l) loc = t * CT_TILE + l; }
  sm[tid] = loc;
  __syncthreads();
  if (tid == 0) { u64 run = 0; for (int i = 0; i < 1024; i++) { u64 v = sm[i]; sm[i] = run; if (v) run = v; } }
  __syncthreads();
  u64 run = sm[tid];
  for (u64 t = a; t < e; t++) { carry_r[t] = run; u32 l = lastchg[t]; if (l) run = t * CT_TILE + l; }
}

__device__ __forceinline__ u32 gstep(bool first_of_stream, bool chg, u32 &m) {
  u32 g;
  if (first_of_stream) { m = 0; return 0; }
  if (chg) { g = enc_size(m + 1); m = 0; }
  else if (m == 258) { g = 5; m = 0; }
  else { g = 0; m++; }
  return g;
}
__device__ __forceinline__ u32 mod259(u64 d) { return (d >> 32) ? (u32)(d % 259ull) : ((u32)d % 259u); }

__global__ void __launch_bounds__(CT_THREADS)
k_cut_b(const u8 *__restrict__ in, u64 n, const u64 *__restrict__ carry_r, u32 *__restrict__ tsum, u8 *__restrict__ gs, u16 *__restrict__ gm) {
  __shared__ i32 sm_i[40];
  __shared__ u32 sm_u[40];
  const u64 t0 = (u64)blockIdx.x * CT_TILE;
  const u32 tid = threadIdx.x;
  const u64 base = t0 + tid * 16;
  u8 b[16];
  load16(in, base, n, b);
  const u8 prev = (base > 0 && base < n) ? in[base - 1] : 0;
  i32 lc = -1;
  {
    u8 pv = prev;
#pragma unroll
    for (int k = 0; k < 16; k++) {
      const u64 p = base + k;
      if (p < n && (p == 0 || b[k] != pv)) lc = (i32)(tid * 16 + k);
      pv = b[k];
    }
  }
  i32 tot;
  const i32 rin = block_excl_max(lc, -1, sm_i, &tot);
  const u64 cr = carry_r[blockIdx.x];
  const u64 r = rin >= 0 ? t0 + (u64)rin : (cr ? cr - 1 : 0);
  u32 local = 0;
  {
    u32 m = (base > 0 && base <= n) ? mod259(base - 1 - r) : 0;
    gm[(size_t)blockIdx.x * CT_THREADS + tid] = (u16)m;
    u8 pv = prev;
#pragma unroll
    for (int k = 0; k < 16; k++) {
      const u64 p = base + k;
      if (p < n) local += gstep(p == 0, b[k] != pv, m);
      pv = b[k];
    }
  }
  gs[(size_t)blockIdx.x * CT_THREADS + tid] = (u8)local;
  u32 total;
  block_excl_add(local, sm_u, &total);
  if (tid == 0) tsum[blockIdx.x] = total;
}

__device__ u64 warp_tile_g(const u8 *__restrict__ in, u64 n, const u8 *__restrict__ gs, const u16 *__restrict__ gm, u64 t, int mode,
                           u64 q, u64 excl, u64 target) {
  const u32 l = lane_id();
  const u64 t0 = t * CT_TILE;
  const u32 w = *reinterpret_cast<const u32 *>(gs + t * CT_THREADS + 4 * l);
  const u32 s0 = w & 255u, s1 = (w >> 8) & 255u, s2 = (w >> 16) & 255u, s3 = w >> 24;
  const u32 c0 = s0, c1 = c0 + s1, c2 = c1 + s2, c3 = c2 + s3;
  const u32 incl = warp_incl_add(c3);
  const u32 before = incl - c3;
  u32 gq;
  u64 run;
  u64 need = 0;
  if (mode == 0) {
    gq = (u32)((q - t0) >> 4);
    const u32 k = gq & 3u;
    const u32 mine = before + (k == 0 ? 0u : k == 1 ? c0 : k == 2 ? c1 : c2);
    run = __shfl_sync(0xffffffffu, mine, gq >> 2);
  } else {
    if (target <= excl) need = 0; else need = target - excl;
    const u32 tot = __shfl_sync(0xffffffffu, incl, 31);
    if (need > tot) return ~0ull;
    const u32 nd = (u32)need;
    int k = -1;
    if (before + c0 >= nd) k = 0; else if (before + c1 >= nd) k = 1; else if (before + c2 >= nd) k = 2; else if (before + c3 >= nd) k = 3;
    const u32 bm = __ballot_sync(0xffffffffu, k >= 0);
    if (!bm) return ~0ull;
    const int src = __ffs(bm) - 1;
    const int ks = __shfl_sync(0xffffffffu, k, src);
    const u32 pre = __shfl_sync(0xffffffffu, before + (ks == 0 ? 0u : ks == 1 ? c0 : ks == 2 ? c1 : c2), src);
    gq = 4u * (u32)src + (u32)ks;
    run = excl + pre;
  }
  const u64 base = t0 + 16ull * gq;
  u8 b[16];
  load16(in, base, n, b);
  u8 pv = (base > 0 && base < n) ? in[base - 1] : 0;
  u32 m = gm[t * CT_THREADS + gq];
  u64 res = ~0ull;
#pragma unroll
  for (int k = 0; k < 16; k++) {
    const u64 p = base + k;
    if (p < n && res == ~0ull) {
      run += gstep(p == 0, b[k] != pv, m);
      if (mode == 0 && p == q) res = run;
      if (mode == 1 && run >= target) res = p;
    }
    pv = b[k];
  }
  return res;
}

__global__ void __launch_bounds__(1024)
k_cut_s2(const u32 *__restrict__ tsum, u64 ntiles, u64 *__restrict__ tincl) {
  __shared__ u64 sm[1024];
  const u32 tid = threadIdx.x;
  const u64 per = (ntiles + 1023) / 1024;
  const u64 a = tid * per, e = min(ntiles, a + per);
  u64 loc = 0;
  for (u64 t = a; t < e; t++) loc += tsum[t];
  sm[tid] = loc;
  __syncthreads();
  if (tid == 0) { u64 run = 0; for (int i = 0; i < 1024; i++) { u64 v = sm[i]; sm[i] = run; run += v; } }
  __syncthreads();
  u64 run = sm[tid];
  for (u64 t = a; t < e; t++) { run += tsum[t]; tincl[t] = run; }
}

__device__ u64 warp_tile(const u8 *__restrict__ in, u64 n, const u64 *__restrict__ carry_r, u64 t, int mode,
                         u64 q, u64 excl, u64 target) {
  const u32 l = lane_id();
  const u64 t0 = t * CT_TILE;
  const u64 base = t0 + l * 64;
  u32 w[16];
#pragma unroll
  for (int v = 0; v < 4; v++) {
    u8 b16[16];
    load16(in, base + 16 * v, n, b16);
#pragma unroll
    for (int k = 0; k < 4; k++) w[4 * v + k] = (u32)b16[4 * k] | ((u32)b16[4 * k + 1] << 8) | ((u32)b16[4 * k + 2] << 16) | ((u32)b16[4 * k + 3] << 24);
  }
  const u8 prev = (base > 0 && base < n) ? in[base - 1] : 0;
  u64 res = ~0ull;
  if (mode == 2) {
    u8 pv = prev;
#pragma unroll
    for (int k = 0; k < 64; k++) {
      const u64 p = base + k;
      const u8 c = (u8)(w[k >> 2] >> (8 * (k & 3)));
      if (p < n && p > q && (p == 0 || c != pv) && res == ~0ull) res = p;
      pv = c;
    }
#pragma unroll
    for (int o = 16; o; o >>= 1) { u64 x = __shfl_xor_sync(0xffffffffu, res, o); res = min(res, x); }
    return res;
  }
  i32 lc = -1;
  {
    u8 pv = prev;
#pragma unroll
    for (int k = 0; k < 64; k++) {
      const u64 p = base + k;
      const u8 c = (u8)(w[k >> 2] >> (8 * (k & 3)));
      if (p < n && (p == 0 || c != pv)) lc = (i32)(l * 64 + k);
      pv = c;
    }
  }
  i32 inc = warp_incl_max(lc);
  i32 rin = __shfl_up_sync(0xffffffffu, inc, 1);
  if (l == 0) rin = -1;
  const u64 cr = carry_r[t];
  const u64 r0 = rin >= 0 ? t0 + (u64)rin : (cr ? cr - 1 : 0);
  const u32 m0 = (base > 0 && base <= n) ? mod259(base - 1 - r0) : 0;
  u32 local = 0;
  {
    u32 m = m0;
    u8 pv = prev;
#pragma unroll 8
    for (int k = 0; k < 64; k++) {
      const u64 p = base + k;
      const u8 c = (u8)(w[k >> 2] >> (8 * (k & 3)));
      if (p < n) local += gstep(p == 0, c != pv, m);
      pv = c;
    }
  }
  const u32 incl = warp_incl_add(local);
  u64 run = excl + (incl - local);
  {
    u32 m = m0;
    u8 pv = prev;
#pragma unroll 8
    for (int k = 0; k < 64; k++) {
      const u64 p = base + k;
      const u8 c = (u8)(w[k >> 2] >> (8 * (k & 3)));
      if (p < n) {
        run += gstep(p == 0, c != pv, m);
        if (mode == 0 && p == q) res = run - excl;
        if (mode == 1 && res == ~0ull && run >= target) res = p;
      }
      pv = c;
    }
  }
#pragma unroll
  for (int o = 16; o; o >>= 1) { u64 x = __shfl_xor_sync(0xffffffffu, res, o); res = min(res, x); }
  return res;
}

__global__ void __launch_bounds__(32)
k_cut_chain(const u8 *__restrict__ in, u64 n, i64 size_hint, int level, i64 win_lo, i64 win_hi,
            const u32 *__restrict__ firstchg, const u64 *__restrict__ carry_r, const u64 *__restrict__ tincl, u64 ntiles,
            const u8 *__restrict__ gs, const u16 *__restrict__ gm,
            B2Chunk *chunks, u32 *n_chunks, u32 max_chunks, u32 *progress, u64 gbase, u64 pos0, u64 stop) {
  const u32 l = lane_id();
  u64 pos = pos0;
  u32 nc = 0;
  for (;;) {
    if (pos >= stop && !(pos0 == 0 && gbase == 0 && n == 0)) break;
    const i64 gpos = (i64)(gbase + pos);
    const i64 rest = size_hint < 0 ? -1 : (gpos <= size_hint ? size_hint - gpos : -1);
    i64 cap = (i64)level * 100000;
    if (rest >= win_lo && rest <= win_hi) cap = rest / 2;
    const u64 avail = n - pos;
    const u64 rawmax = (u64)(10 * cap);
    const u64 limit = avail < rawmax ? avail : rawmax;
    const u64 need = cap > 5 ? (u64)(cap - 5) : 0;
    u64 len = limit;
    if (need == 0) len = 0;
    else if (limit > 0) {
      const u64 s = pos, end_max = pos + limit;
      u64 e1 = ~0ull;
      {
        u64 t = s / CT_TILE;
        {
          const u64 p = s + 1 + l;
          const bool chg = p < n && in[p] != in[p - 1];
          const u32 bm = __ballot_sync(0xffffffffu, chg);
          if (bm) e1 = s + 1 + (u64)(__ffs(bm) - 1);
        }
        if (e1 == ~0ull) e1 = warp_tile(in, n, carry_r, t, 2, s, 0, 0);
        if (e1 == ~0ull) {
          for (u64 tb = t + 1; tb < ntiles && e1 == ~0ull; tb += 32) {
            const u64 tt = tb + l;
            const u32 f = tt < ntiles ? firstchg[tt] : NONE32;
            const u32 m = __ballot_sync(0xffffffffu, f != NONE32);
            if (m) { const int k = __ffs(m) - 1; const u32 fk = __shfl_sync(0xffffffffu, f, k); e1 = (tb + k) * CT_TILE + fk; }
            if (tb * CT_TILE >= end_max) break;
          }
        }
        if (e1 == ~0ull) e1 = n;
      }
      const u64 run_end = e1 < end_max ? e1 : end_max;
      const u64 jstar = (need + 4) / 5;
      const u64 pstar = s + 259 * jstar;
      if (pstar < run_end) len = pstar - s + 1;
      else if (e1 >= end_max) len = limit;
      else {
        const u64 L1 = e1 - s;
        const u64 A = 5 * ((L1 - 1) / 259) + enc_size((u32)((L1 - 1) % 259) + 1);
        if (A >= need) len = e1 - s + 1;
        else {
          const u64 te = e1 / CT_TILE;
          const u64 excl_e = te ? tincl[te - 1] : 0;
          const u64 Ge1 = excl_e + warp_tile_g(in, n, gs, gm, te, 0, e1, 0, 0);
          const u64 Gt = Ge1 + (need - A);
          u64 lo = te, hi = ntiles;
          { const u64 wend = end_max / CT_TILE + 1; if (wend < hi) hi = wend; }
          while (lo < hi) {
            const u64 span = hi - lo, step = (span + 31) / 32;
            const u64 upto = (u64)(l + 1) * step;
            const u64 pr = lo + (upto < span ? upto : span) - 1;
            const u32 m = __ballot_sync(0xffffffffu, tincl[pr] >= Gt);
            if (m == 0) { lo = hi; break; }
            const int k = __ffs(m) - 1;
            hi = __shfl_sync(0xffffffffu, pr, k);
            lo = lo + (u64)k * step;
          }
          if (lo < ntiles && lo * CT_TILE < end_max) {
            const u64 excl = lo ? tincl[lo - 1] : 0;
            const u64 p = warp_tile_g(in, n, gs, gm, lo, 1, 0, excl, Gt);
            if (p != ~0ull && p < end_max) len = p - s + 1;
          }
        }
      }
    }
    if (l == 0 && nc < max_chunks) { chunks[nc].start = pos; chunks[nc].len = (u32)len; chunks[nc].cap = (u32)cap; chunks[nc].pad = 0; chunks[nc].pad2 = 0; }
    nc++;
    if (l == 0 && progress) { __threadfence(); *(volatile u32 *)progress = nc < max_chunks ? nc : max_chunks; }
    pos += len;
    if (pos >= n) break;
    if (len == 0) break;
  }
  if (l == 0) {
    n_chunks[0] = nc;
    n_chunks[2] = (u32)pos; n_chunks[3] = (u32)(pos >> 32);
    if (progress) { __threadfence(); ((volatile u32 *)progress)[1] = 1u; }
  }
}

int b2k_cut_scans(cudaStream_t st, const u8 *d_in, u64 n, B2CutWork *w) {
  const u64 ntiles = (n + CT_TILE - 1) / CT_TILE;
  if (ntiles) {
    k_cut_a<<<(u32)ntiles, CT_THREADS, 0, st>>>(d_in, n, w->firstchg, w->lastchg);
    k_cut_s1<<<1, 1024, 0, st>>>(w->lastchg, ntiles, w->carry_r);
    k_cut_b<<<(u32)ntiles, CT_THREADS, 0, st>>>(d_in, n, w->carry_r, w->tsum, w->gs, w->gm);
    k_cut_s2<<<1, 1024, 0, st>>>(w->tsum, ntiles, w->tincl);
    B2_CUDA_CHECK(cudaGetLastError());
  }
  return 0;
}

int b2k_cut_chain(cudaStream_t st, const u8 *d_in, u64 n, i64 size_hint, int level, i64 win_lo, i64 win_hi,
                  B2Chunk *d_chunks, u32 *d_n_chunks, u32 max_chunks, B2CutWork *w, u32 *d_progress, cudaEvent_t ev_chain_starts,
                  u64 gbase, u64 pos0, u64 stop) {
  const u64 ntiles = (n + CT_TILE - 1) / CT_TILE;
  if (d_progress) B2_CUDA_CHECK(cudaMemsetAsync(d_progress, 0, 2 * sizeof(u32), st));
  if (ev_chain_starts) B2_CUDA_CHECK(cudaEventRecord(ev_chain_starts, st));
  k_cut_chain<<<1, 32, 0, st>>>(d_in, n, size_hint, level, win_lo, win_hi, w->firstchg, w->carry_r, w->tincl, ntiles, w->gs, w->gm,
                                d_chunks, d_n_chunks, max_chunks, d_progress, gbase, pos0, stop);
  B2_CUDA_CHECK(cudaGetLastError());
  return 0;
}

int b2k_cut(cudaStream_t st, const u8 *d_in, u64 n, i64 size_hint, int level, i64 win_lo, i64 win_hi,
            B2Chunk *d_chunks, u32 *d_n_chunks, u32 max_chunks, B2CutWork *w, u32 *d_progress, cudaEvent_t ev_chain_starts) {
  B2_TRY_K(b2k_cut_scans(st, d_in, n, w));
  return b2k_cut_chain(st, d_in, n, size_hint, level, win_lo, win_hi, d_chunks, d_n_chunks, max_chunks, w, d_progress, ev_chain_starts,
                       0, 0, n);
}
```

zip-ada_b200/csrc/b2_kernels.h:

```cpp
#pragma once
#include "b2_common.cuh"

struct B2Chunk { u64 start; u32 len; u32 cap; u32 pad; u32 pad2; };

struct B2CrcTables {
  u32 byte_tab[256];
  u32 xp_thread[1024];
  u32 x_tile;
  u32 xinv_a[1024];
  u32 xinv_b[16];
  u32 pw2[32];
};

struct B2SortTile { u32 job; u32 start; };
struct B2SortTileRR { u32 job; u32 start; u32 prev; u32 pad; };

struct B2SortStats {
  u64 scatter_launches;
  u64 scatter_elems;
  double scatter_ms;
  u64 rounds;
  u64 sorted_elems_round0;
  u64 sorted_elems_later;
  double sort_ms;
  u64 launches;
};

struct B2CutWork { u32 *firstchg, *lastchg, *tsum; u64 *carry_r, *tincl; u8 *gs; u16 *gm; };
int b2k_cut(cudaStream_t st, const u8 *d_in, u64 n, i64 size_hint, int level, i64 win_lo, i64 win_hi,
            B2Chunk *d_chunks, u32 *d_n_chunks, u32 max_chunks, B2CutWork *w, u32 *d_progress, cudaEvent_t ev_chain_starts);
int b2k_cut_scans(cudaStream_t st, const u8 *d_in, u64 n, B2CutWork *w);
int b2k_cut_chain(cudaStream_t st, const u8 *d_in, u64 n, i64 size_hint, int level, i64 win_lo, i64 win_hi,
                  B2Chunk *d_chunks, u32 *d_n_chunks, u32 max_chunks, B2CutWork *w, u32 *d_progress, cudaEvent_t ev_chain_starts,
                  u64 gbase, u64 pos0, u64 stop);
#define B2_SEG_GAVE_UP 0xFFFFFFFDu
#define B2_SEG_PENDING 0xFEFEFEFEu
int b2k_segment(cudaStream_t st, const u8 *d_in, const B2Chunk *d_chunks, u32 n_chunks, const double *d_T,
                u32 *d_seg, u32 *d_nseg, const u32 *d_progress);
void b2k_make_crc_tables(B2CrcTables *t);
int b2k_rle1(cudaStream_t st, const u8 *d_in, B2Job *d_jobs, u32 n_jobs, u8 *d_text, const B2CrcTables *d_ct);

struct B2SortJob { u32 job, tile0, ntiles, pad; };
struct B2ConcatItem { u64 src_word; u64 nbits; u64 dst_bit; };
struct B2StreamEnd { u64 out_off; u64 end_bit; u32 crc; u32 pad; };
struct B2PackItem { u64 src_off; u64 dst_off; u64 len; };

struct B2SortCtx {
  u64 *keysA, *keysB;
  u32 *valsA, *valsB, *rank, *grp;
  u32 *slotA, *slotB, *sa_full, *d_tile_cnt;
  B2SortTile *d_tiles;
  B2SortJob *d_sj;
  u32 *d_hist, *d_digit_base;
  B2SortTileRR *d_tiles_rr;
  u32 *d_ticket;
  const B2Job *h_jobs;
  u32 max_used;
  int sym_bits;
  i32 *d_tile_head, *d_carry;
  u32 *d_unsorted, *h_unsorted;
  size_t max_tiles, max_jobs;
  bool timing;
  B2SortStats stats;
};

#define LL_MAXCODE 20

#ifdef __cplusplus
#include <vector>
int b2k_bwt_batch(B2SortCtx *cx, cudaStream_t st, B2Job *d_jobs, const std::vector<u32> &job_ids,
                  const std::vector<u32> &job_n, const u8 *d_text, u8 *d_bwt);
#endif
#define B2_MTF_TILE 4096
#define B2_SORT_TILE 2048
#define B2_MTF_SEG 32768
int b2k_mtf(cudaStream_t st, B2Job *d_jobs, u32 n_jobs, const B2SortTile *d_tiles, u32 n_tiles,
            const B2SortTile *d_segs, u32 n_segs_small, u32 n_segs_mid, u32 n_segs, const u8 *d_bwt, u32 *d_m16, u32 *d_m256,
            u32 *d_tilemask, u8 *d_idx, u16 *d_mtf);
int b2k_entropy(cudaStream_t st, B2Job *d_jobs, u32 n_jobs, u32 max_groups_per_job, u32 total_groups,
                const u16 *d_mtf, u16 *d_ghist, u8 *d_gdist, u32 *d_rank3, u32 *d_rank4, u8 *d_sel, u8 *d_selprev,
                u32 *d_gpack, u16 *d_gselcost,
                u32 *d_hist, u32 *d_leaves, u32 *d_wl, u8 *d_lens, u32 *d_stat, u32 *d_selcost, u32 *d_cost, u32 *d_low,
                int level, u32 max_alpha, u32 *d_activated, u64 *launches);
int b2k_bits_layout(cudaStream_t st, B2Job *d_jobs, u32 n_jobs, u64 *d_total_words);
int b2k_pack(cudaStream_t st, const B2Job *d_jobs, u32 n_jobs, const u16 *d_mtf, const u8 *d_sel, const u8 *d_lens,
             u8 *d_selpos, u32 *d_bits, int level, u32 total_groups);
int b2k_concat(cudaStream_t st, const B2ConcatItem *d_items, u32 n_items, const u32 *d_bits, u32 *d_out);
int b2k_stream_ends(cudaStream_t st, const B2StreamEnd *d_ends, u32 n, int level, u32 *d_out);
int b2k_pack_streams(cudaStream_t st, const B2PackItem *d_items, u32 n, const u8 *d_src, u8 *d_dst);

#define B2_ZIP_TILE 65536
struct B2ZipCrcTables {
  u32 byte_tab[256];
  u32 xp_thread[1024];
  u32 pw2[48];
};
struct B2ZipTile { u64 begin; u64 end; };
struct B2ZipEntry { u64 len; u32 tile0; u32 n_tiles; };
struct B2ZipCopy { u64 src_off; u64 dst_off; u32 len; u32 which; };
void b2k_make_zipcrc_tables(B2ZipCrcTables *t);
int b2k_zipcrc(cudaStream_t st, const u8 *d_in, const B2ZipTile *d_tiles, u32 n_tiles, const B2ZipEntry *d_ents, u32 n_entries,
               const B2ZipCrcTables *d_zt, u32 *d_partial, u32 *d_crc);
int b2k_zip_gather(cudaStream_t st, const B2ZipCopy *d_items, u32 n, const u8 *d_src0, const u8 *d_src1, u8 *d_dst);

struct B2VBlock {
  u64 start_bit;
  u64 end_bit;
  u64 raw_len;
  u64 raw_off;
  u32 stored_crc, computed_crc, n_rle, orig_ptr, status, pad;
};
int b2k_verify_find(cudaStream_t st, const u8 *d_stream, u64 n_bytes, u64 *d_cand, u32 *d_n_cand, u32 cap);
int b2k_verify_decode(cudaStream_t st, const u8 *d_stream, u64 n_bytes, B2VBlock *d_blocks, u32 n_blocks, u32 max_n, u32 *d_link, u8 *d_lcol,
                      u8 *d_rle, u8 *d_sel, const u32 *d_crc_tab);
int b2k_verify_compare(cudaStream_t st, const B2VBlock *d_blocks, const u32 *d_chain, u32 n_chain, u32 max_n, const u8 *d_rle,
                       const u8 *d_expect, u64 expect_n, unsigned long long *d_first_bad);
```

zip-ada_b200/csrc/b2_segment.cu:

```cuda
#include "b2_common.cuh"
#include "b2_kernels.h"

#define SEG_WINDOW 16000
#define SG_THREADS 256
#define SG_WARPS (SG_THREADS / 32)

typedef long long i64s;

__device__ __forceinline__ double pow2d(int e) { return __longlong_as_double((long long)(e + 1023) << 52); }

template <int N> struct PF { i64s a[N]; };

template <int N> __device__ __forceinline__ i64s pf_pick(const PF<N> &g, i64s idx) {
  const int r = (int)(idx & (N - 1));
  if (N == 2) return r ? g.a[1] : g.a[0];
  const i64s lo = (r & 1) ? g.a[1] : g.a[0];
  const i64s hi = (r & 1) ? g.a[N - 1] : g.a[N - 2];
  return (r & 2) ? hi : lo;
}
template <int N> __device__ __forceinline__ PF<N> pf_compose(const PF<N> &f, const PF<N> &g) {
  PF<N> r;
#pragma unroll
  for (int i = 0; i < N; i++) r.a[i] = f.a[i] + pf_pick<N>(g, (i64s)i + f.a[i]);
  return r;
}
__device__ __forceinline__ i64s pf_apply(i64s k, double x, bool coarse) {
  const double fl = floor(x);
  const i64s X = (i64s)fl;
  const double fr = x - fl;
  if (!coarse) {
    const i64s m = X + (fr > 0.5 ? 1 : 0);
    return k + m + (((fr == 0.5) && ((k + m) & 1)) ? 1 : 0);
  }
  const i64s Y = X + (k & 1);
  const bool odd = (Y & 1) != 0;
  const i64s q = (k >> 1) + (Y >> 1) + ((odd && fr > 0.0) ? 1 : 0);
  return 2 * (q + ((odd && fr == 0.0 && (q & 1)) ? 1 : 0));
}
template <int N> __device__ __forceinline__ PF<N> pf_term(double x, bool coarse) {
  const double fl = floor(x);
  const i64s X = (i64s)fl;
  const double fr = x - fl;
  PF<N> f;
  if (N == 2 || !coarse) {
    const i64s m = X + (fr > 0.5 ? 1 : 0);
    const bool tie = fr == 0.5;
#pragma unroll
    for (int r = 0; r < N; r++) f.a[r] = m + ((tie && ((r + m) & 1)) ? 1 : 0);
  } else {
#pragma unroll
    for (int b = 0; b < 2; b++) {
      const i64s Y = X + b;
      const bool odd = (Y & 1) != 0;
      const i64s m = (Y >> 1) + ((odd && fr > 0.0) ? 1 : 0);
      const bool tie = odd && fr == 0.0;
#pragma unroll
      for (int qp = 0; qp < 2; qp++) f.a[(2 * qp + b) & (N - 1)] = 2 * (m + ((tie && ((qp + m) & 1)) ? 1 : 0)) - b;
    }
  }
  return f;
}

struct SegSmem {
  u32 F[256];
  u32 Hn[SG_WARPS][256];
  u32 Ho[SG_WARPS][256];
  u16 Pn[SG_WARPS][256];
  u16 Po[SG_WARPS][256];
  double terms[SG_THREADS * 4];
  double series[SG_THREADS];
  i64s wtot[SG_WARPS][4];
  double cutval[2];
  double restartE;
  u32 first[2];
  u32 firstbad;
  u8 bn[SG_THREADS], bo[SG_THREADS];
  u32 pm_lt[8][32], pm_le[8][32];
  double entropy;
};

template <int N> __device__ __forceinline__ void seg_scan(SegSmem &S, double E, double scale, double split, bool part,
                                                          const double (&d)[4], i64s &kb, i64s &k, bool &mybad) {
  const u32 l = lane_id(), w = warp_id();
  const i64s K0 = (i64s)(E * scale);
  u32 coarse = 0;
  PF<N> inc, mine_f;
  {
    double v = E;
#pragma unroll
    for (int j = 0; j < 4; j++) {
      v += d[j];
      const bool cj = N == 4 && part && v >= split;
      coarse |= (u32)cj << j;
      const PF<N> fj = pf_term<N>(part ? d[j] * scale : 0.0, cj);
      inc = j == 0 ? fj : pf_compose<N>(inc, fj);
    }
    mine_f = inc;
  }
#pragma unroll
  for (int o = 1; o < 32; o <<= 1) {
    PF<N> nb;
#pragma unroll
    for (int r = 0; r < N; r++) nb.a[r] = __shfl_up_sync(0xffffffffu, inc.a[r], o);
    if (l >= (u32)o) inc = pf_compose<N>(nb, inc);
  }
  if (l == 31) {
#pragma unroll
    for (int r = 0; r < N; r++) S.wtot[w][r] = inc.a[r];
  }
  PF<N> excl;
#pragma unroll
  for (int r = 0; r < N; r++) { excl.a[r] = __shfl_up_sync(0xffffffffu, inc.a[r], 1); if (l == 0) excl.a[r] = 0; }
  __syncthreads();
  PF<N> pre;
#pragma unroll
  for (int r = 0; r < N; r++) pre.a[r] = 0;
  for (u32 ww = 0; ww < w; ww++) {
    PF<N> g;
#pragma unroll
    for (int r = 0; r < N; r++) g.a[r] = S.wtot[ww][r];
    pre = pf_compose<N>(pre, g);
  }
  pre = pf_compose<N>(pre, excl);
  kb = K0 + pf_pick<N>(pre, K0);
  if (N == 2) {
    k = K0 + pf_pick<N>(pf_compose<N>(pre, mine_f), K0);
    mybad = false;
    return;
  }
  k = kb;
  const i64s lo = 1ll << 52, mid = 1ll << 53, hi = N == 2 ? mid : (1ll << 54);
  mybad = false;
#pragma unroll
  for (int j = 0; j < 4; j++) {
    const bool cj = ((coarse >> j) & 1u) != 0;
    k = pf_apply(k, d[j] * scale, cj);
    mybad = mybad || k < lo || k >= hi || (N == 4 && ((k >= mid) != cj));
  }
  mybad = mybad && part;
}

__global__ void __launch_bounds__(SG_THREADS, 3)
k_segment(const u8 *__restrict__ in, const B2Chunk *chunks, u32 n_chunks,
          const double *__restrict__ T, u32 *__restrict__ seg, u32 *__restrict__ nseg, const u32 *progress) {
  __shared__ SegSmem S;
  const u32 c = blockIdx.x;
  if (c >= n_chunks) return;
  const u32 tid = threadIdx.x, l = lane_id(), w = warp_id();
  if (progress) {
    if (tid == 0) {
      u32 state = 2;
      for (u32 spins = 0; spins < 8000000u; spins++) {
        const u32 done = ((const volatile u32 *)progress)[1];
        const u32 ready = ((const volatile u32 *)progress)[0];
        if (ready > c) { state = 1; break; }
        if (done) { state = 0; break; }
        __nanosleep(400);
      }
      S.first[0] = state;
      if (state == 2) { nseg[2 * c] = B2_SEG_GAVE_UP; nseg[2 * c + 1] = B2_SEG_GAVE_UP; }
    }
    __syncthreads();
    const u32 state = S.first[0];
    __syncthreads();
    if (state != 1) return;
    __threadfence();
  }
  const u32 lt = (1u << l) - 1u;
  const u8 *buf = in + __ldcg(&chunks[c].start);
  const i32 len = (i32)__ldcg(&chunks[c].len);
  const double thr[2] = {(double)0.6f, (double)0.4f};
  const i32 ithr[2] = {4000, 8000};
  i32 index_mark[2] = {1, 1};
  double mark[2] = {0.0, 0.0};
  u32 cnt[2] = {0, 0};
  u32 *out[2] = {seg + (size_t)(2 * c) * B2_MAX_SEG, seg + (size_t)(2 * c + 1) * B2_MAX_SEG};
  const bool act[2] = {len > SEG_WINDOW + ithr[0], len > SEG_WINDOW + ithr[1]};
  if (act[0] || act[1]) {
    S.F[tid] = 0;
    for (int i = tid; i < SG_WARPS * 256; i += SG_THREADS) { (&S.Hn[0][0])[i] = 0; (&S.Ho[0][0])[i] = 0; }
    __syncthreads();
    for (i32 i = tid; i < SEG_WINDOW; i += SG_THREADS) atomicAdd(&S.F[buf[i]], 1u);
    __syncthreads();
    if (w == 0) {
      double e = 0.0;
      for (int g = 0; g < 8; g++) {
        const u32 f = S.F[g * 32 + l];
        const double tv = T[f];
        for (int k = 0; k < 32; k++) {
          const u32 fk = __shfl_sync(0xffffffffu, f, k);
          const double tk = __shfl_sync(0xffffffffu, tv, k);
          if (fk > 0) e = __dadd_rn(e, tk);
        }
      }
      if (l == 0) S.entropy = e;
    }
    __syncthreads();
    double entropy = S.entropy;
    mark[0] = entropy; mark[1] = entropy;
    if (w == 0) {
#pragma unroll
      for (int q = 0; q < 8; q++) {
        const int lo = 4 * q;
        const int a_lt = (int)l - lo, a_le = (int)l + 1 - lo;
        S.pm_lt[q][l] = a_lt >= 4 ? 0xFFFFFFFFu : (a_lt <= 0 ? 0u : ((1u << (8 * a_lt)) - 1u));
        S.pm_le[q][l] = a_le >= 4 ? 0xFFFFFFFFu : (a_le <= 0 ? 0u : ((1u << (8 * a_le)) - 1u));
      }
    }
    __syncthreads();
    const u32 *rown = reinterpret_cast<const u32 *>(S.bn + 32 * w);
    const u32 *rowo = reinterpret_cast<const u32 *>(S.bo + 32 * w);
    u32 pre_n = (SEG_WINDOW + (i32)tid < len) ? buf[SEG_WINDOW + tid] : 0u;
    u32 pre_o = (SEG_WINDOW + (i32)tid < len) ? buf[tid] : 0u;
    for (i32 i0 = SEG_WINDOW; i0 < len; i0 += SG_THREADS) {
      const i32 i = i0 + (i32)tid;
      const bool valid = i < len;
      const u32 bn = pre_n, bo = pre_o;
      {
        const i32 i2 = i + SG_THREADS;
        const bool v2 = i2 < len;
        pre_n = v2 ? buf[i2] : 0u;
        pre_o = v2 ? buf[i2 - SEG_WINDOW] : 0u;
      }
      const int steps = min(SG_THREADS, len - i0);
      S.bn[tid] = (u8)bn; S.bo[tid] = (u8)bo;
      if (tid < 2) S.first[tid] = 0xFFFFFFFFu;
      const u32 key_n = valid ? bn : (256u + l), key_o = valid ? bo : (512u + l);
      const u32 peers_n = __match_any_sync(0xffffffffu, key_n), peers_o = __match_any_sync(0xffffffffu, key_o);
      const u32 c_nn = __popc(peers_n & lt);
      const u32 c_oo = __popc(peers_o & lt);
      const bool lead_n = valid && c_nn == 0, lead_o = valid && c_oo == 0;
      if (lead_n) S.Hn[w][bn] = __popc(peers_n);
      if (lead_o) S.Ho[w][bo] = __popc(peers_o);
      __syncthreads();
      i32 dF;
      {
        u32 rn = 0, ro = 0;
#pragma unroll
        for (int ww = 0; ww < SG_WARPS; ww++) {
          S.Pn[ww][tid] = (u16)rn; S.Po[ww][tid] = (u16)ro;
          rn += S.Hn[ww][tid]; ro += S.Ho[ww][tid];
        }
        dF = (i32)rn - (i32)ro;
      }
      __syncthreads();
      const u32 sp_n = bn * 0x01010101u, sp_o = bo * 0x01010101u;
      u32 c_on = 0, c_no = 0;
#pragma unroll
      for (int q = 0; q < 8; q++) {
        c_on += __popc(__vcmpeq4(rowo[q], sp_n) & S.pm_lt[q][l]);
        c_no += __popc(__vcmpeq4(rown[q], sp_o) & S.pm_le[q][l]);
      }
      c_on >>= 3; c_no >>= 3;
      u32 fnb = 0, fob = 1;
      if (valid) {
        fnb = S.F[bn] + (S.Pn[w][bn] + c_nn) - (S.Po[w][bn] + c_on);
        fob = S.F[bo] + (S.Pn[w][bo] + c_no) - (S.Po[w][bo] + c_oo);
      }
      const double c1 = T[fnb], c2 = T[fnb + 1], c3 = T[fob], c4 = T[fob - 1];
      double mine = 0.0;
      u32 start = 0;
      double E = entropy;
      int attempts = 0;
      bool finished = false;
      while (!finished) {
        if (E >= 0x1p-12 && E < 8.0 && attempts < 12) {
          const int eb = (int)((__double_as_longlong(E) >> 52) & 0x7FF) - 1023;
          const double blo = pow2d(eb);
          const bool one = (E - blo >= 0.75) && (2.0 * blo - E > 0.75);
          const int B = one ? eb : ((E < 1.5 * blo) ? eb - 1 : eb);
          const double scale = pow2d(52 - B), inv = pow2d(B - 52);
          const bool part = valid && tid >= start;
          if (tid == 0) S.firstbad = 0xFFFFFFFFu;
          const double d[4] = {-c1, c2, -c3, c4};
          i64s kb, k;
          bool mybad;
          if (one) seg_scan<2>(S, E, scale, pow2d(B + 1), part, d, kb, k, mybad);
          else seg_scan<4>(S, E, scale, pow2d(B + 1), part, d, kb, k, mybad);
          if (__syncthreads_or(mybad) == 0) {
            if (part) mine = (double)k * inv;
            if ((int)tid == steps - 1) S.entropy = mine;
            finished = true;
          } else {
            if (mybad) atomicMin(&S.firstbad, tid);
            __syncthreads();
            const u32 fb = S.firstbad;
            if (part && tid < fb) mine = (double)k * inv;
            if (tid == fb) {
              double ee = (double)kb * inv;
              ee = __dsub_rn(ee, c1);
              ee = __dadd_rn(ee, c2);
              ee = __dsub_rn(ee, c3);
              ee = __dadd_rn(ee, c4);
              mine = ee;
              S.restartE = ee;
              if ((int)tid == steps - 1) S.entropy = ee;
            }
            __syncthreads();
            E = S.restartE;
            start = fb + 1;
            attempts++;
            if ((int)start >= steps) finished = true;
          }
        } else {
          S.terms[tid * 4 + 0] = c1; S.terms[tid * 4 + 1] = c2; S.terms[tid * 4 + 2] = c3; S.terms[tid * 4 + 3] = c4;
          __syncthreads();
          if (w == 0) {
            double e = E;
            for (int k = (int)start; k < steps; k++) {
              const double2 ab = *reinterpret_cast<const double2 *>(&S.terms[k * 4]);
              const double2 cd = *reinterpret_cast<const double2 *>(&S.terms[k * 4 + 2]);
              e = __dsub_rn(e, ab.x);
              e = __dadd_rn(e, ab.y);
              e = __dsub_rn(e, cd.x);
              e = __dadd_rn(e, cd.y);
              if (l == 0) S.series[k] = e;
            }
            if (l == 0) S.entropy = e;
          }
          __syncthreads();
          if (tid >= start) mine = S.series[tid];
          finished = true;
        }
      }
      const i32 sp = i + 1 - SEG_WINDOW;
      bool maybe[2];
#pragma unroll
      for (int p = 0; p < 2; p++) {
        maybe[p] = act[p] && (i0 + steps - SEG_WINDOW - index_mark[p] > ithr[p]);
        if (maybe[p] && valid && fabs(__dsub_rn(mine, mark[p])) > thr[p] && (sp - index_mark[p] > ithr[p])) atomicMin(&S.first[p], tid);
      }
      if (lead_n) S.Hn[w][bn] = 0;
      if (lead_o) S.Ho[w][bo] = 0;
      __syncthreads();
      S.F[tid] = (u32)((i32)S.F[tid] + dF);
#pragma unroll
      for (int p = 0; p < 2; p++) if (maybe[p] && S.first[p] == tid) S.cutval[p] = mine;
      __syncthreads();
      entropy = S.entropy;
#pragma unroll
      for (int p = 0; p < 2; p++) {
        if (maybe[p] && S.first[p] != 0xFFFFFFFFu) {
          const i32 seg_point = i0 + (i32)S.first[p] + 1 - SEG_WINDOW;
          if (tid == 0 && cnt[p] < B2_MAX_SEG - 1) out[p][cnt[p]] = (u32)seg_point;
          cnt[p]++;
          index_mark[p] = seg_point;
          mark[p] = S.cutval[p];
        }
      }
      __syncthreads();
    }
  }
  if (tid == 0) {
    for (int k = 0; k < 2; k++) {
      if (len > 0) { if (cnt[k] < B2_MAX_SEG) out[k][cnt[k]] = (u32)len; cnt[k]++; }
    }
    __threadfence();
    nseg[2 * c] = cnt[0]; nseg[2 * c + 1] = cnt[1];
  }
}

int b2k_segment(cudaStream_t st, const u8 *d_in, const B2Chunk *d_chunks, u32 n_chunks, const double *d_T,
                u32 *d_seg, u32 *d_nseg, const u32 *d_progress) {
  if (n_chunks == 0) return 0;
  k_segment<<<n_chunks, SG_THREADS, 0, st>>>(d_in, d_chunks, n_chunks, d_T, d_seg, d_nseg, d_progress);
  B2_CUDA_CHECK(cudaGetLastError());
  return 0;
}
```

Measured before the change: 1827.

## Replace streamed segmentation overlap with warp-pipelined producer/consumer segment kernel

```diff
diff --git a/zip-ada_b200/csrc/b2_api.cu b/zip-ada_b200/csrc/b2_api.cu
--- a/zip-ada_b200/csrc/b2_api.cu
+++ b/zip-ada_b200/csrc/b2_api.cu
@@ -128,8 +128,6 @@
   b2_progress_fn progress = nullptr;
   void *progress_user = nullptr;
   cudaStream_t st = nullptr;
-  cudaStream_t st2 = nullptr;
-  cudaEvent_t ev_fork = nullptr, ev_join = nullptr;
   int timing = 0;
   DevBuf<B2CrcTables> d_ct;
   DevBuf<double> d_T;
@@ -163,7 +161,6 @@
   B2SortStats sort_stats;
   bool batch_positions_fixed = false;
   size_t batch_positions = 1536ull << 20;
-  size_t first_batch_positions = ~(size_t)0;
   size_t batch_jobs_max = 65535;
   int n_workspaces = 1;
   u64 launches_other = 0;
@@ -438,20 +435,17 @@
   e->stats.kernel_launches = e->launches_other + e->sort_stats.launches;
 }
 
-int encode_chunks(b2_encoder *e, const u8 *d_in, std::vector<StreamDesc> &streams, std::vector<u32> &chunk_stream, bool followed,
-                  ShardState *sh);
+int encode_chunks(b2_encoder *e, const u8 *d_in, std::vector<StreamDesc> &streams, std::vector<u32> &chunk_stream, ShardState *sh);
 
 int encode_streams(b2_encoder *e, const u8 *d_in, std::vector<StreamDesc> &streams) {
   cudaStream_t st = e->st;
   const int level = e->level;
-  B2_CUDA_CHECK(cudaStreamSynchronize(e->st2));
   e->shard.open = e->shard.cut = e->shard.encoded = false;
   e->trace.clear(); e->chunks.clear(); e->nseg.clear(); e->seg.clear();
   i64 win_lo, win_hi;
   balance_window(level, win_lo, win_hi);
   const i64 full_cap = (i64)level * 100000;
   std::vector<u32> chunk_stream;
-  bool followed = false;
   {
     StageTimer tm(e, st, e->ev, &e->stats.stage_ms[0]);
     const u64 small_limit = (u64)((win_lo / 2 - 16) * 4 / 5);
@@ -471,22 +465,8 @@
         B2_TRY(e->d_cut_carry.ensure(ct)); B2_TRY(e->d_cut_tincl.ensure(ct));
         B2_TRY(e->d_cut_gs.ensure(ct * 128)); B2_TRY(e->d_cut_gm.ensure(ct * 128));
         B2CutWork cw{e->d_cut_first.p, e->d_cut_last.p, e->d_cut_tsum.p, e->d_cut_carry.p, e->d_cut_tincl.p, e->d_cut_gs.p, e->d_cut_gm.p};
-        const bool follow = level == 9 && streams.size() == 1 && e->timing < 2;
-        if (follow) {
-          B2_TRY(e->d_seg.ensure((size_t)max_chunks * 2 * B2_MAX_SEG));
-          B2_TRY(e->d_nseg.ensure((size_t)max_chunks * 2));
-          B2_CUDA_CHECK(cudaMemsetAsync(e->d_nseg.p, 0xFE, (size_t)max_chunks * 2 * sizeof(u32), st));
-        }
-        B2_TRY(b2k_cut(st, d_in + S.off, S.n, S.hint, level, win_lo, win_hi, e->d_chunks.p, e->d_scalars.p, max_chunks, &cw,
-                       follow ? e->d_scalars.p + 12 : nullptr, follow ? e->ev_fork : nullptr));
+        B2_TRY(b2k_cut(st, d_in + S.off, S.n, S.hint, level, win_lo, win_hi, e->d_chunks.p, e->d_scalars.p, max_chunks, &cw));
         e->launches_other += 5;
-        if (follow) {
-          B2_CUDA_CHECK(cudaStreamWaitEvent(e->st2, e->ev_fork, 0));
-          B2_TRY(b2k_segment(e->st2, d_in + S.off, e->d_chunks.p, max_chunks, e->d_T.p, e->d_seg.p, e->d_nseg.p, e->d_scalars.p + 12));
-          B2_CUDA_CHECK(cudaEventRecord(e->ev_join, e->st2));
-          e->launches_other += 1;
-          followed = true;
-        }
         u32 nc = 0;
         B2_CUDA_CHECK(cudaMemcpyAsync(&nc, e->d_scalars.p, sizeof(u32), cudaMemcpyDeviceToHost, st));
         B2_CUDA_CHECK(cudaStreamSynchronize(st));
@@ -501,11 +481,10 @@
       for (u32 c = 0; c < S.n_chunks; c++) chunk_stream.push_back((u32)si);
     }
   }
-  return encode_chunks(e, d_in, streams, chunk_stream, followed, nullptr);
-}
-
-int encode_chunks(b2_encoder *e, const u8 *d_in, std::vector<StreamDesc> &streams, std::vector<u32> &chunk_stream, bool followed,
-                  ShardState *sh) {
+  return encode_chunks(e, d_in, streams, chunk_stream, nullptr);
+}
+
+int encode_chunks(b2_encoder *e, const u8 *d_in, std::vector<StreamDesc> &streams, std::vector<u32> &chunk_stream, ShardState *sh) {
   cudaStream_t st = e->st;
   const int level = e->level;
   const u32 n_chunks = (u32)e->chunks.size();
@@ -514,59 +493,28 @@
   if (sh) { sh->cands.assign((size_t)n_chunks * 4, ShardCand{0, 0, 0, 0, 0, 0}); sh->n_tactics.assign(n_chunks, 0); }
   {
     StageTimer tm(e, st, e->ev, &e->stats.stage_ms[0]);
-    if (!followed) {
-      B2_TRY(e->d_chunks.ensure(n_chunks));
-      B2_CUDA_CHECK(cudaMemcpyAsync(e->d_chunks.p, e->chunks.data(), n_chunks * sizeof(B2Chunk), cudaMemcpyHostToDevice, st));
-    }
+    B2_TRY(e->d_chunks.ensure(n_chunks));
+    B2_CUDA_CHECK(cudaMemcpyAsync(e->d_chunks.p, e->chunks.data(), n_chunks * sizeof(B2Chunk), cudaMemcpyHostToDevice, st));
     if (level == 9) {
       e->nseg.assign((size_t)n_chunks * 2, 0);
       e->seg.assign((size_t)n_chunks * 2, std::vector<u32>());
-      if (!followed) {
-        B2_TRY(e->d_seg.ensure((size_t)n_chunks * 2 * B2_MAX_SEG));
-        B2_TRY(e->d_nseg.ensure((size_t)n_chunks * 2));
-        B2_TRY(b2k_segment(st, d_in, e->d_chunks.p, n_chunks, e->d_T.p, e->d_seg.p, e->d_nseg.p, nullptr));
-        e->launches_other += 1;
+      B2_TRY(e->d_seg.ensure((size_t)n_chunks * 2 * B2_MAX_SEG));
+      B2_TRY(e->d_nseg.ensure((size_t)n_chunks * 2));
+      B2_TRY(b2k_segment(st, d_in, e->d_chunks.p, n_chunks, e->d_T.p, e->d_seg.p, e->d_nseg.p));
+      e->launches_other += 1;
+      B2_CUDA_CHECK(cudaMemcpyAsync(e->nseg.data(), e->d_nseg.p, 2 * (size_t)n_chunks * sizeof(u32), cudaMemcpyDeviceToHost, st));
+      B2_CUDA_CHECK(cudaStreamSynchronize(st));
+      for (size_t k = 0; k < 2 * (size_t)n_chunks; k++) {
+        const u32 ns = e->nseg[k];
+        if (ns > B2_MAX_SEG) B2_FAIL(B2_ERR_INTERNAL, "segment table overflow");
+        if (ns > 1) {
+          e->seg[k].resize(ns);
+          B2_CUDA_CHECK(cudaMemcpyAsync(e->seg[k].data(), e->d_seg.p + k * B2_MAX_SEG, ns * sizeof(u32), cudaMemcpyDeviceToHost, st));
+        }
       }
     }
     B2_CUDA_CHECK(cudaStreamSynchronize(st));
   }
-  u32 seg_have = 0;
-  auto fetch_seg = [&](u32 upto) -> int {
-    if (level != 9 || upto <= seg_have) return 0;
-    upto = std::min(n_chunks, std::max(upto, seg_have + 64));
-    for (u32 tries = 0;; tries++) {
-      B2_CUDA_CHECK(cudaMemcpyAsync(e->nseg.data() + 2 * (size_t)seg_have, e->d_nseg.p + 2 * (size_t)seg_have,
-                                    2 * (size_t)(upto - seg_have) * sizeof(u32), cudaMemcpyDeviceToHost, st));
-      B2_CUDA_CHECK(cudaStreamSynchronize(st));
-      bool all = true, gave_up = false;
-      for (u32 k = 2 * seg_have; k < 2 * upto; k++) {
-        if (e->nseg[k] == B2_SEG_PENDING) { all = false; break; }
-        if (e->nseg[k] == B2_SEG_GAVE_UP) gave_up = true;
-      }
-      if (all && gave_up) {
-        B2_CUDA_CHECK(cudaStreamSynchronize(e->st2));
-        B2_CUDA_CHECK(cudaMemcpyAsync(e->d_chunks.p, e->chunks.data(), n_chunks * sizeof(B2Chunk), cudaMemcpyHostToDevice, st));
-        B2_TRY(b2k_segment(st, d_in, e->d_chunks.p, n_chunks, e->d_T.p, e->d_seg.p, e->d_nseg.p, nullptr));
-        e->launches_other += 1;
-        followed = false;
-        continue;
-      }
-      if (all) break;
-      if (!followed || tries > 2000000u) B2_FAIL(B2_ERR_INTERNAL, "segmentation results missing");
-      std::this_thread::sleep_for(std::chrono::microseconds(50));
-    }
-    for (u32 k = 2 * seg_have; k < 2 * upto; k++) {
-      const u32 ns = e->nseg[k];
-      if (ns > B2_MAX_SEG) B2_FAIL(B2_ERR_INTERNAL, "segment table overflow");
-      if (ns > 1) {
-        e->seg[k].resize(ns);
-        B2_CUDA_CHECK(cudaMemcpyAsync(e->seg[k].data(), e->d_seg.p + (size_t)k * B2_MAX_SEG, ns * sizeof(u32), cudaMemcpyDeviceToHost, st));
-      }
-    }
-    B2_CUDA_CHECK(cudaStreamSynchronize(st));
-    seg_have = upto;
-    return 0;
-  };
   u64 out_total = 0;
   for (auto &S : streams) {
     S.out_off = out_total;
@@ -722,11 +670,9 @@
   int plan_rc = 0;
   std::string plan_msg;
   {
-    u32 published = 0;
     auto publish = [&](Batch &&bt) {
       { std::lock_guard<std::mutex> lk(bmu); batches.push_back(std::move(bt)); }
       bcv.notify_all();
-      published++;
     };
     Batch cur; cur.c0 = 0;
     u64 positions = 0;
@@ -736,10 +682,8 @@
       P.start = e->chunks[c].start; P.len = e->chunks[c].len; P.cap = e->chunks[c].cap;
       P.n_seg[0] = P.n_seg[1] = 0;
       u64 addpos = 0;
-      if ((plan_rc = fetch_seg(c + 1))) break;
       if ((plan_rc = plan_chunk(e, c, P, add, cur.jobs.size(), addpos))) break;
-      const size_t limit = (followed && published == 0) ? std::min(e->first_batch_positions, batch_limit) : batch_limit;
-      if (!cur.jobs.empty() && (positions + addpos > limit || cur.jobs.size() + add.size() > e->batch_jobs_max)) {
+      if (!cur.jobs.empty() && (positions + addpos > batch_limit || cur.jobs.size() + add.size() > e->batch_jobs_max)) {
         cur.c1 = c;
         publish(std::move(cur));
         cur = Batch(); cur.c0 = c; positions = 0;
@@ -780,7 +724,6 @@
     }
   }
   for (auto &t : th) t.join();
-  if (followed) B2_CUDA_CHECK(cudaStreamSynchronize(e->st2));
   (void)out_words_needed;
   if (err) { g_last_error = err_msg; return err; }
   if (!sh) {
@@ -867,14 +810,10 @@
   memset(&e->stats, 0, sizeof e->stats);
   memset(&e->sort_stats, 0, sizeof e->sort_stats);
   if (const char *s = getenv("B2GPU_BATCH_POSITIONS")) { long long v = atoll(s); if (v >= (1 << 20)) { e->batch_positions = (size_t)std::min<long long>(v, 3ll << 30); e->batch_positions_fixed = true; } }
-  if (const char *s = getenv("B2GPU_FIRST_BATCH_POSITIONS")) { long long v = atoll(s); if (v >= (1 << 20)) e->first_batch_positions = (size_t)v; }
   if (const char *s = getenv("B2GPU_BATCH_JOBS")) { long long v = atoll(s); if (v >= 8) e->batch_jobs_max = (size_t)std::min<long long>(v, 65535); }
   if (const char *s = getenv("B2GPU_PIPELINE")) { int v = atoi(s); if (v >= 1 && v <= 8) e->n_workspaces = v; }
   auto init = [&]() -> int {
     B2_CUDA_CHECK(cudaStreamCreateWithFlags(&e->st, cudaStreamNonBlocking));
-    B2_CUDA_CHECK(cudaStreamCreateWithFlags(&e->st2, cudaStreamNonBlocking));
-    B2_CUDA_CHECK(cudaEventCreateWithFlags(&e->ev_fork, cudaEventDisableTiming));
-    B2_CUDA_CHECK(cudaEventCreateWithFlags(&e->ev_join, cudaEventDisableTiming));
     B2_CUDA_CHECK(cudaEventCreate(&e->ev[0])); B2_CUDA_CHECK(cudaEventCreate(&e->ev[1]));
     B2_CUDA_CHECK(cudaEventCreate(&e->ev_call[0])); B2_CUDA_CHECK(cudaEventCreate(&e->ev_call[1]));
     for (int i = 0; i < e->n_workspaces; i++) {
@@ -920,9 +859,6 @@
   if (e->ev[1]) cudaEventDestroy(e->ev[1]);
   if (e->ev_call[0]) cudaEventDestroy(e->ev_call[0]);
   if (e->ev_call[1]) cudaEventDestroy(e->ev_call[1]);
-  if (e->st2) { cudaStreamSynchronize(e->st2); cudaStreamDestroy(e->st2); }
-  if (e->ev_fork) cudaEventDestroy(e->ev_fork);
-  if (e->ev_join) cudaEventDestroy(e->ev_join);
   if (e->st) cudaStreamDestroy(e->st);
   delete e;
 }
@@ -1044,7 +980,6 @@
                   uint64_t stream_size, int64_t size_hint, uint64_t own_end) {
   if (!e || (n_local && !in) || base + n_local > stream_size || own_end > stream_size || own_end < base) B2_FAIL(B2_ERR_ARGUMENT, "bad argument");
   B2_CUDA_CHECK(cudaSetDevice(e->device));
-  B2_CUDA_CHECK(cudaStreamSynchronize(e->st2));
   ShardState &sh = e->shard;
   sh.open = sh.cut = sh.encoded = false;
   sh.base = base; sh.n_local = n_local; sh.stream_n = stream_size; sh.hint = size_hint; sh.own_end = own_end;
@@ -1082,23 +1017,11 @@
   const u32 max_chunks = (u32)(own / (40000ull * level) + 16);
   B2_TRY(e->d_chunks.ensure(max_chunks));
   B2CutWork cw{e->d_cut_first.p, e->d_cut_last.p, e->d_cut_tsum.p, e->d_cut_carry.p, e->d_cut_tincl.p, e->d_cut_gs.p, e->d_cut_gm.p};
-  const bool follow = level == 9 && e->timing < 2;
-  if (level == 9) {
-    B2_TRY(e->d_seg.ensure((size_t)max_chunks * 2 * B2_MAX_SEG));
-    B2_TRY(e->d_nseg.ensure((size_t)max_chunks * 2));
-    B2_CUDA_CHECK(cudaMemsetAsync(e->d_nseg.p, 0xFE, (size_t)max_chunks * 2 * sizeof(u32), st));
-  }
   const bool last = sh.own_end >= sh.stream_n;
   const u64 stop = last ? sh.n_local : sh.own_end - sh.base;
   B2_TRY(b2k_cut_chain(st, sh.d_in, sh.n_local, sh.hint, level, win_lo, win_hi, e->d_chunks.p, e->d_scalars.p, max_chunks, &cw,
-                       follow ? e->d_scalars.p + 12 : nullptr, follow ? e->ev_fork : nullptr, sh.base, entry - sh.base, stop));
+                       sh.base, entry - sh.base, stop));
   e->launches_other += 1;
-  if (follow) {
-    B2_CUDA_CHECK(cudaStreamWaitEvent(e->st2, e->ev_fork, 0));
-    B2_TRY(b2k_segment(e->st2, sh.d_in, e->d_chunks.p, max_chunks, e->d_T.p, e->d_seg.p, e->d_nseg.p, e->d_scalars.p + 12));
-    B2_CUDA_CHECK(cudaEventRecord(e->ev_join, e->st2));
-    e->launches_other += 1;
-  }
   u32 sc[4] = {0, 0, 0, 0};
   B2_CUDA_CHECK(cudaMemcpyAsync(sc, e->d_scalars.p, sizeof sc, cudaMemcpyDeviceToHost, st));
   B2_CUDA_CHECK(cudaStreamSynchronize(st));
@@ -1123,8 +1046,7 @@
   streams[0] = StreamDesc{0, sh.n_local, sh.hint, 0, 0, 0, nc};
   e->stats.streams++; e->stats.input_bytes += sh.handoff - sh.entry;
   std::vector<u32> chunk_stream(nc, 0u);
-  const bool followed = e->level == 9 && e->timing < 2;
-  B2_TRY(encode_chunks(e, sh.d_in, streams, chunk_stream, followed, &sh));
+  B2_TRY(encode_chunks(e, sh.d_in, streams, chunk_stream, &sh));
   for (u32 phase0 = 0; phase0 < 8; phase0++) {
     u64 total = 0; u32 rot = 0, fold = 0, ph = phase0;
     for (u32 c = 0; c < nc; c++) {
diff --git a/zip-ada_b200/csrc/b2_chunks.cu b/zip-ada_b200/csrc/b2_chunks.cu
--- a/zip-ada_b200/csrc/b2_chunks.cu
+++ b/zip-ada_b200/csrc/b2_chunks.cu
@@ -266,7 +266,7 @@
 k_cut_chain(const u8 *__restrict__ in, u64 n, i64 size_hint, int level, i64 win_lo, i64 win_hi,
             const u32 *__restrict__ firstchg, const u64 *__restrict__ carry_r, const u64 *__restrict__ tincl, u64 ntiles,
             const u8 *__restrict__ gs, const u16 *__restrict__ gm,
-            B2Chunk *chunks, u32 *n_chunks, u32 max_chunks, u32 *progress, u64 gbase, u64 pos0, u64 stop) {
+            B2Chunk *chunks, u32 *n_chunks, u32 max_chunks, u64 gbase, u64 pos0, u64 stop) {
   const u32 l = lane_id();
   u64 pos = pos0;
   u32 nc = 0;
@@ -341,7 +341,6 @@
     }
     if (l == 0 && nc < max_chunks) { chunks[nc].start = pos; chunks[nc].len = (u32)len; chunks[nc].cap = (u32)cap; chunks[nc].pad = 0; chunks[nc].pad2 = 0; }
     nc++;
-    if (l == 0 && progress) { __threadfence(); *(volatile u32 *)progress = nc < max_chunks ? nc : max_chunks; }
     pos += len;
     if (pos >= n) break;
     if (len == 0) break;
@@ -349,7 +348,6 @@
   if (l == 0) {
     n_chunks[0] = nc;
     n_chunks[2] = (u32)pos; n_chunks[3] = (u32)(pos >> 32);
-    if (progress) { __threadfence(); ((volatile u32 *)progress)[1] = 1u; }
   }
 }
 
@@ -366,20 +364,16 @@
 }
 
 int b2k_cut_chain(cudaStream_t st, const u8 *d_in, u64 n, i64 size_hint, int level, i64 win_lo, i64 win_hi,
-                  B2Chunk *d_chunks, u32 *d_n_chunks, u32 max_chunks, B2CutWork *w, u32 *d_progress, cudaEvent_t ev_chain_starts,
-                  u64 gbase, u64 pos0, u64 stop) {
+                  B2Chunk *d_chunks, u32 *d_n_chunks, u32 max_chunks, B2CutWork *w, u64 gbase, u64 pos0, u64 stop) {
   const u64 ntiles = (n + CT_TILE - 1) / CT_TILE;
-  if (d_progress) B2_CUDA_CHECK(cudaMemsetAsync(d_progress, 0, 2 * sizeof(u32), st));
-  if (ev_chain_starts) B2_CUDA_CHECK(cudaEventRecord(ev_chain_starts, st));
   k_cut_chain<<<1, 32, 0, st>>>(d_in, n, size_hint, level, win_lo, win_hi, w->firstchg, w->carry_r, w->tincl, ntiles, w->gs, w->gm,
-                                d_chunks, d_n_chunks, max_chunks, d_progress, gbase, pos0, stop);
+                                d_chunks, d_n_chunks, max_chunks, gbase, pos0, stop);
   B2_CUDA_CHECK(cudaGetLastError());
   return 0;
 }
 
 int b2k_cut(cudaStream_t st, const u8 *d_in, u64 n, i64 size_hint, int level, i64 win_lo, i64 win_hi,
-            B2Chunk *d_chunks, u32 *d_n_chunks, u32 max_chunks, B2CutWork *w, u32 *d_progress, cudaEvent_t ev_chain_starts) {
+            B2Chunk *d_chunks, u32 *d_n_chunks, u32 max_chunks, B2CutWork *w) {
   B2_TRY_K(b2k_cut_scans(st, d_in, n, w));
-  return b2k_cut_chain(st, d_in, n, size_hint, level, win_lo, win_hi, d_chunks, d_n_chunks, max_chunks, w, d_progress, ev_chain_starts,
-                       0, 0, n);
-}
+  return b2k_cut_chain(st, d_in, n, size_hint, level, win_lo, win_hi, d_chunks, d_n_chunks, max_chunks, w, 0, 0, n);
+}
diff --git a/zip-ada_b200/csrc/b2_kernels.h b/zip-ada_b200/csrc/b2_kernels.h
--- a/zip-ada_b200/csrc/b2_kernels.h
+++ b/zip-ada_b200/csrc/b2_kernels.h
@@ -28,15 +28,12 @@
 
 struct B2CutWork { u32 *firstchg, *lastchg, *tsum; u64 *carry_r, *tincl; u8 *gs; u16 *gm; };
 int b2k_cut(cudaStream_t st, const u8 *d_in, u64 n, i64 size_hint, int level, i64 win_lo, i64 win_hi,
-            B2Chunk *d_chunks, u32 *d_n_chunks, u32 max_chunks, B2CutWork *w, u32 *d_progress, cudaEvent_t ev_chain_starts);
+            B2Chunk *d_chunks, u32 *d_n_chunks, u32 max_chunks, B2CutWork *w);
 int b2k_cut_scans(cudaStream_t st, const u8 *d_in, u64 n, B2CutWork *w);
 int b2k_cut_chain(cudaStream_t st, const u8 *d_in, u64 n, i64 size_hint, int level, i64 win_lo, i64 win_hi,
-                  B2Chunk *d_chunks, u32 *d_n_chunks, u32 max_chunks, B2CutWork *w, u32 *d_progress, cudaEvent_t ev_chain_starts,
-                  u64 gbase, u64 pos0, u64 stop);
-#define B2_SEG_GAVE_UP 0xFFFFFFFDu
-#define B2_SEG_PENDING 0xFEFEFEFEu
+                  B2Chunk *d_chunks, u32 *d_n_chunks, u32 max_chunks, B2CutWork *w, u64 gbase, u64 pos0, u64 stop);
 int b2k_segment(cudaStream_t st, const u8 *d_in, const B2Chunk *d_chunks, u32 n_chunks, const double *d_T,
-                u32 *d_seg, u32 *d_nseg, const u32 *d_progress);
+                u32 *d_seg, u32 *d_nseg);
 void b2k_make_crc_tables(B2CrcTables *t);
 int b2k_rle1(cudaStream_t st, const u8 *d_in, B2Job *d_jobs, u32 n_jobs, u8 *d_text, const B2CrcTables *d_ct);
 
diff --git a/zip-ada_b200/csrc/b2_segment.cu b/zip-ada_b200/csrc/b2_segment.cu
--- a/zip-ada_b200/csrc/b2_segment.cu
+++ b/zip-ada_b200/csrc/b2_segment.cu
@@ -2,368 +2,189 @@
 #include "b2_kernels.h"
 
 #define SEG_WINDOW 16000
-#define SG_THREADS 256
-#define SG_WARPS (SG_THREADS / 32)
 
-typedef long long i64s;
+#define SG_SLOTS 16
+#define SG_THREADS 96
 
-__device__ __forceinline__ double pow2d(int e) { return __longlong_as_double((long long)(e + 1023) << 52); }
-
-template <int N> struct PF { i64s a[N]; };
-
-template <int N> __device__ __forceinline__ i64s pf_pick(const PF<N> &g, i64s idx) {
-  const int r = (int)(idx & (N - 1));
-  if (N == 2) return r ? g.a[1] : g.a[0];
-  const i64s lo = (r & 1) ? g.a[1] : g.a[0];
-  const i64s hi = (r & 1) ? g.a[N - 1] : g.a[N - 2];
-  return (r & 2) ? hi : lo;
-}
-template <int N> __device__ __forceinline__ PF<N> pf_compose(const PF<N> &f, const PF<N> &g) {
-  PF<N> r;
-#pragma unroll
-  for (int i = 0; i < N; i++) r.a[i] = f.a[i] + pf_pick<N>(g, (i64s)i + f.a[i]);
-  return r;
-}
-__device__ __forceinline__ i64s pf_apply(i64s k, double x, bool coarse) {
-  const double fl = floor(x);
-  const i64s X = (i64s)fl;
-  const double fr = x - fl;
-  if (!coarse) {
-    const i64s m = X + (fr > 0.5 ? 1 : 0);
-    return k + m + (((fr == 0.5) && ((k + m) & 1)) ? 1 : 0);
-  }
-  const i64s Y = X + (k & 1);
-  const bool odd = (Y & 1) != 0;
-  const i64s q = (k >> 1) + (Y >> 1) + ((odd && fr > 0.0) ? 1 : 0);
-  return 2 * (q + ((odd && fr == 0.0 && (q & 1)) ? 1 : 0));
-}
-template <int N> __device__ __forceinline__ PF<N> pf_term(double x, bool coarse) {
-  const double fl = floor(x);
-  const i64s X = (i64s)fl;
-  const double fr = x - fl;
-  PF<N> f;
-  if (N == 2 || !coarse) {
-    const i64s m = X + (fr > 0.5 ? 1 : 0);
-    const bool tie = fr == 0.5;
-#pragma unroll
-    for (int r = 0; r < N; r++) f.a[r] = m + ((tie && ((r + m) & 1)) ? 1 : 0);
-  } else {
-#pragma unroll
-    for (int b = 0; b < 2; b++) {
-      const i64s Y = X + b;
-      const bool odd = (Y & 1) != 0;
-      const i64s m = (Y >> 1) + ((odd && fr > 0.0) ? 1 : 0);
-      const bool tie = odd && fr == 0.0;
-#pragma unroll
-      for (int qp = 0; qp < 2; qp++) f.a[(2 * qp + b) & (N - 1)] = 2 * (m + ((tie && ((qp + m) & 1)) ? 1 : 0)) - b;
+__global__ void __launch_bounds__(SG_THREADS)
+k_segment(const u8 *__restrict__ in, const B2Chunk *__restrict__ chunks, u32 n_chunks,
+          const double *__restrict__ T, u32 *__restrict__ seg, u32 *__restrict__ nseg) {
+  __shared__ u32 F[256];
+  __shared__ double2 ring[SG_SLOTS][32][2];
+  __shared__ double ringE[SG_SLOTS][32];
+  __shared__ u32 produced, consumed, tested;
+  __shared__ double entropy0;
+  __shared__ __align__(4) u8 rown[64], rowo[64];
+  const u32 c = blockIdx.x;
+  if (c >= n_chunks) return;
+  const u32 tid = threadIdx.x, l = tid & 31u, w = tid >> 5;
+  const u8 *buf = in + chunks[c].start;
+  const i32 len = (i32)chunks[c].len;
+  const i32 ithr0 = 4000, ithr1 = 8000;
+  const bool act0 = len > SEG_WINDOW + ithr0, act1 = len > SEG_WINDOW + ithr1;
+  u32 *out0 = seg + (size_t)(2 * c) * B2_MAX_SEG, *out1 = seg + (size_t)(2 * c + 1) * B2_MAX_SEG;
+  if (!act0) {
+    if (tid == 0) {
+      const u32 k = len > 0 ? 1u : 0u;
+      if (k) { out0[0] = (u32)len; out1[0] = (u32)len; }
+      nseg[2 * c] = k; nseg[2 * c + 1] = k;
     }
-  }
-  return f;
-}
-
-struct SegSmem {
-  u32 F[256];
-  u32 Hn[SG_WARPS][256];
-  u32 Ho[SG_WARPS][256];
-  u16 Pn[SG_WARPS][256];
-  u16 Po[SG_WARPS][256];
-  double terms[SG_THREADS * 4];
-  double series[SG_THREADS];
-  i64s wtot[SG_WARPS][4];
-  double cutval[2];
-  double restartE;
-  u32 first[2];
-  u32 firstbad;
-  u8 bn[SG_THREADS], bo[SG_THREADS];
-  u32 pm_lt[8][32], pm_le[8][32];
-  double entropy;
-};
-
-template <int N> __device__ __forceinline__ void seg_scan(SegSmem &S, double E, double scale, double split, bool part,
-                                                          const double (&d)[4], i64s &kb, i64s &k, bool &mybad) {
-  const u32 l = lane_id(), w = warp_id();
-  const i64s K0 = (i64s)(E * scale);
-  u32 coarse = 0;
-  PF<N> inc, mine_f;
-  {
-    double v = E;
-#pragma unroll
-    for (int j = 0; j < 4; j++) {
-      v += d[j];
-      const bool cj = N == 4 && part && v >= split;
-      coarse |= (u32)cj << j;
-      const PF<N> fj = pf_term<N>(part ? d[j] * scale : 0.0, cj);
-      inc = j == 0 ? fj : pf_compose<N>(inc, fj);
-    }
-    mine_f = inc;
-  }
-#pragma unroll
-  for (int o = 1; o < 32; o <<= 1) {
-    PF<N> nb;
-#pragma unroll
-    for (int r = 0; r < N; r++) nb.a[r] = __shfl_up_sync(0xffffffffu, inc.a[r], o);
-    if (l >= (u32)o) inc = pf_compose<N>(nb, inc);
-  }
-  if (l == 31) {
-#pragma unroll
-    for (int r = 0; r < N; r++) S.wtot[w][r] = inc.a[r];
-  }
-  PF<N> excl;
-#pragma unroll
-  for (int r = 0; r < N; r++) { excl.a[r] = __shfl_up_sync(0xffffffffu, inc.a[r], 1); if (l == 0) excl.a[r] = 0; }
-  __syncthreads();
-  PF<N> pre;
-#pragma unroll
-  for (int r = 0; r < N; r++) pre.a[r] = 0;
-  for (u32 ww = 0; ww < w; ww++) {
-    PF<N> g;
-#pragma unroll
-    for (int r = 0; r < N; r++) g.a[r] = S.wtot[ww][r];
-    pre = pf_compose<N>(pre, g);
-  }
-  pre = pf_compose<N>(pre, excl);
-  kb = K0 + pf_pick<N>(pre, K0);
-  if (N == 2) {
-    k = K0 + pf_pick<N>(pf_compose<N>(pre, mine_f), K0);
-    mybad = false;
     return;
   }
-  k = kb;
-  const i64s lo = 1ll << 52, mid = 1ll << 53, hi = N == 2 ? mid : (1ll << 54);
-  mybad = false;
-#pragma unroll
-  for (int j = 0; j < 4; j++) {
-    const bool cj = ((coarse >> j) & 1u) != 0;
-    k = pf_apply(k, d[j] * scale, cj);
-    mybad = mybad || k < lo || k >= hi || (N == 4 && ((k >= mid) != cj));
-  }
-  mybad = mybad && part;
-}
-
-__global__ void __launch_bounds__(SG_THREADS, 3)
-k_segment(const u8 *__restrict__ in, const B2Chunk *chunks, u32 n_chunks,
-          const double *__restrict__ T, u32 *__restrict__ seg, u32 *__restrict__ nseg, const u32 *progress) {
-  __shared__ SegSmem S;
-  const u32 c = blockIdx.x;
-  if (c >= n_chunks) return;
-  const u32 tid = threadIdx.x, l = lane_id(), w = warp_id();
-  if (progress) {
-    if (tid == 0) {
-      u32 state = 2;
-      for (u32 spins = 0; spins < 8000000u; spins++) {
-        const u32 done = ((const volatile u32 *)progress)[1];
-        const u32 ready = ((const volatile u32 *)progress)[0];
-        if (ready > c) { state = 1; break; }
-        if (done) { state = 0; break; }
-        __nanosleep(400);
-      }
-      S.first[0] = state;
-      if (state == 2) { nseg[2 * c] = B2_SEG_GAVE_UP; nseg[2 * c + 1] = B2_SEG_GAVE_UP; }
-    }
-    __syncthreads();
-    const u32 state = S.first[0];
-    __syncthreads();
-    if (state != 1) return;
-    __threadfence();
-  }
-  const u32 lt = (1u << l) - 1u;
-  const u8 *buf = in + __ldcg(&chunks[c].start);
-  const i32 len = (i32)__ldcg(&chunks[c].len);
-  const double thr[2] = {(double)0.6f, (double)0.4f};
-  const i32 ithr[2] = {4000, 8000};
-  i32 index_mark[2] = {1, 1};
-  double mark[2] = {0.0, 0.0};
-  u32 cnt[2] = {0, 0};
-  u32 *out[2] = {seg + (size_t)(2 * c) * B2_MAX_SEG, seg + (size_t)(2 * c + 1) * B2_MAX_SEG};
-  const bool act[2] = {len > SEG_WINDOW + ithr[0], len > SEG_WINDOW + ithr[1]};
-  if (act[0] || act[1]) {
-    S.F[tid] = 0;
-    for (int i = tid; i < SG_WARPS * 256; i += SG_THREADS) { (&S.Hn[0][0])[i] = 0; (&S.Ho[0][0])[i] = 0; }
-    __syncthreads();
-    for (i32 i = tid; i < SEG_WINDOW; i += SG_THREADS) atomicAdd(&S.F[buf[i]], 1u);
-    __syncthreads();
-    if (w == 0) {
-      double e = 0.0;
-      for (int g = 0; g < 8; g++) {
-        const u32 f = S.F[g * 32 + l];
-        const double tv = T[f];
-        for (int k = 0; k < 32; k++) {
-          const u32 fk = __shfl_sync(0xffffffffu, f, k);
-          const double tk = __shfl_sync(0xffffffffu, tv, k);
-          if (fk > 0) e = __dadd_rn(e, tk);
-        }
-      }
-      if (l == 0) S.entropy = e;
-    }
-    __syncthreads();
-    double entropy = S.entropy;
-    mark[0] = entropy; mark[1] = entropy;
-    if (w == 0) {
-#pragma unroll
-      for (int q = 0; q < 8; q++) {
-        const int lo = 4 * q;
-        const int a_lt = (int)l - lo, a_le = (int)l + 1 - lo;
-        S.pm_lt[q][l] = a_lt >= 4 ? 0xFFFFFFFFu : (a_lt <= 0 ? 0u : ((1u << (8 * a_lt)) - 1u));
-        S.pm_le[q][l] = a_le >= 4 ? 0xFFFFFFFFu : (a_le <= 0 ? 0u : ((1u << (8 * a_le)) - 1u));
+  const i32 n = len - SEG_WINDOW;
+  const i32 ng = (n + 31) / 32;
+  for (u32 b = tid; b < 256; b += SG_THREADS) F[b] = 0;
+  if (tid == 0) { produced = 0; consumed = 0; tested = 0; }
+  __syncthreads();
+  for (i32 i = tid; i < SEG_WINDOW; i += SG_THREADS) atomicAdd(&F[buf[i]], 1u);
+  __syncthreads();
+  if (w == 0) {
+    double e = 0.0;
+    for (int g = 0; g < 8; g++) {
+      const u32 f = F[g * 32 + l];
+      const double tv = T[f];
+      for (int k = 0; k < 32; k++) {
+        const u32 fk = __shfl_sync(0xffffffffu, f, k);
+        const double tk = __shfl_sync(0xffffffffu, tv, k);
+        if (fk > 0) e = __dadd_rn(e, tk);
       }
     }
-    __syncthreads();
-    const u32 *rown = reinterpret_cast<const u32 *>(S.bn + 32 * w);
-    const u32 *rowo = reinterpret_cast<const u32 *>(S.bo + 32 * w);
-    u32 pre_n = (SEG_WINDOW + (i32)tid < len) ? buf[SEG_WINDOW + tid] : 0u;
-    u32 pre_o = (SEG_WINDOW + (i32)tid < len) ? buf[tid] : 0u;
-    for (i32 i0 = SEG_WINDOW; i0 < len; i0 += SG_THREADS) {
-      const i32 i = i0 + (i32)tid;
-      const bool valid = i < len;
-      const u32 bn = pre_n, bo = pre_o;
-      {
-        const i32 i2 = i + SG_THREADS;
-        const bool v2 = i2 < len;
-        pre_n = v2 ? buf[i2] : 0u;
-        pre_o = v2 ? buf[i2 - SEG_WINDOW] : 0u;
+    if (l == 0) entropy0 = e;
+  }
+  __syncthreads();
+  if (w == 0) {
+    if (l != 0) return;
+    double E = entropy0;
+    const volatile u32 *vprod = &produced, *vtest = &tested;
+    volatile u32 *vcons = &consumed;
+    for (i32 g = 0; g < ng; g++) {
+      while ((i32)*vprod <= g || g - (i32)*vtest >= SG_SLOTS) {}
+      __threadfence_block();
+      const double2 (*slot)[2] = ring[g % SG_SLOTS];
+      double *es = ringE[g % SG_SLOTS];
+      auto step = [&](int k) {
+        const double2 a = slot[k][0], b = slot[k][1];
+        E = __dsub_rn(E, a.x);
+        E = __dadd_rn(E, a.y);
+        E = __dsub_rn(E, b.x);
+        E = __dadd_rn(E, b.y);
+        es[k] = E;
+      };
+      const i32 steps = min(32, n - 32 * g);
+      if (steps == 32) {
+#pragma unroll
+        for (int k = 0; k < 32; k++) step(k);
+      } else {
+        for (int k = 0; k < steps; k++) step(k);
       }
-      const int steps = min(SG_THREADS, len - i0);
-      S.bn[tid] = (u8)bn; S.bo[tid] = (u8)bo;
-      if (tid < 2) S.first[tid] = 0xFFFFFFFFu;
-      const u32 key_n = valid ? bn : (256u + l), key_o = valid ? bo : (512u + l);
-      const u32 peers_n = __match_any_sync(0xffffffffu, key_n), peers_o = __match_any_sync(0xffffffffu, key_o);
-      const u32 c_nn = __popc(peers_n & lt);
-      const u32 c_oo = __popc(peers_o & lt);
-      const bool lead_n = valid && c_nn == 0, lead_o = valid && c_oo == 0;
-      if (lead_n) S.Hn[w][bn] = __popc(peers_n);
-      if (lead_o) S.Ho[w][bo] = __popc(peers_o);
-      __syncthreads();
-      i32 dF;
-      {
-        u32 rn = 0, ro = 0;
+      __threadfence_block();
+      *vcons = (u32)(g + 1);
+    }
+    return;
+  }
+  if (w == 2) {
+    const double thr0 = (double)0.6f, thr1 = (double)0.4f;
+    double mark0 = entropy0, mark1 = entropy0;
+    i32 im0 = 1, im1 = 1;
+    u32 cnt0 = 0, cnt1 = 0;
+    const volatile u32 *vcons = &consumed;
+    volatile u32 *vtest = &tested;
+    for (i32 g = 0; g < ng; g++) {
+      if (l == 0) while ((i32)*vcons <= g) __nanosleep(256);
+      __syncwarp();
+      __threadfence_block();
+      const i32 sp = 32 * g + (i32)l + 1;
+      const bool valid = sp <= n;
+      const double e = valid ? ringE[g % SG_SLOTS][l] : 0.0;
+      __syncwarp();
+      if (l == 0) { __threadfence_block(); *vtest = (u32)(g + 1); }
+      const u32 h0 = __ballot_sync(0xffffffffu, valid && sp - im0 > ithr0 && fabs(__dsub_rn(e, mark0)) > thr0);
+      const u32 h1 = __ballot_sync(0xffffffffu, valid && act1 && sp - im1 > ithr1 && fabs(__dsub_rn(e, mark1)) > thr1);
+      if (h0) {
+        const int k = __ffs(h0) - 1;
+        mark0 = __shfl_sync(0xffffffffu, e, k); im0 = 32 * g + k + 1;
+        if (l == 0 && cnt0 < B2_MAX_SEG - 1) out0[cnt0] = (u32)im0;
+        cnt0++;
+      }
+      if (h1) {
+        const int k = __ffs(h1) - 1;
+        mark1 = __shfl_sync(0xffffffffu, e, k); im1 = 32 * g + k + 1;
+        if (l == 0 && cnt1 < B2_MAX_SEG - 1) out1[cnt1] = (u32)im1;
+        cnt1++;
+      }
+    }
+    if (l == 0) {
+      if (cnt0 < B2_MAX_SEG) out0[cnt0] = (u32)len;
+      if (cnt1 < B2_MAX_SEG) out1[cnt1] = (u32)len;
+      nseg[2 * c] = cnt0 + 1; nseg[2 * c + 1] = cnt1 + 1;
+    }
+    return;
+  }
+  const u8 *bo_p = buf, *bn_p = buf + SEG_WINDOW;
+  const volatile u32 *vcons = &consumed;
+  volatile u32 *vprod = &produced;
+  u32 nb[2], ob[2];
 #pragma unroll
-        for (int ww = 0; ww < SG_WARPS; ww++) {
-          S.Pn[ww][tid] = (u16)rn; S.Po[ww][tid] = (u16)ro;
-          rn += S.Hn[ww][tid]; ro += S.Ho[ww][tid];
-        }
-        dF = (i32)rn - (i32)ro;
+  for (int h = 0; h < 2; h++) {
+    const i32 j = 32 * h + (i32)l;
+    nb[h] = j < n ? bn_p[j] : 0u; ob[h] = j < n ? bo_p[j] : 0u;
+  }
+  for (i32 g = 0; g < ng; g += 2) {
+    u32 bn[2], bo[2];
+    bool valid[2];
+#pragma unroll
+    for (int h = 0; h < 2; h++) {
+      const i32 j = 32 * (g + h) + (i32)l;
+      valid[h] = j < n;
+      bn[h] = nb[h]; bo[h] = ob[h];
+      if (j + 64 < n) { nb[h] = bn_p[j + 64]; ob[h] = bo_p[j + 64]; }
+      rown[32 * h + l] = (u8)bn[h]; rowo[32 * h + l] = (u8)bo[h];
+    }
+    __syncwarp();
+    u32 fnb[2], fob[2];
+#pragma unroll
+    for (int h = 0; h < 2; h++) {
+      const u32 spn = bn[h] * 0x01010101u, spo = bo[h] * 0x01010101u;
+      u32 c_nn = 0, c_on = 0, c_no = 0, c_oo = 0;
+#pragma unroll
+      for (int q = 0; q < 8 * (h + 1); q++) {
+        const int a = 32 * h + (int)l - 4 * q;
+        const u32 lt = a >= 4 ? 0xFFFFFFFFu : (a <= 0 ? 0u : ((1u << (8 * a)) - 1u));
+        const u32 wn = reinterpret_cast<const u32 *>(rown)[q], wo = reinterpret_cast<const u32 *>(rowo)[q];
+        c_nn += __popc(__vcmpeq4(wn, spn) & lt); c_on += __popc(__vcmpeq4(wo, spn) & lt);
+        c_no += __popc(__vcmpeq4(wn, spo) & lt); c_oo += __popc(__vcmpeq4(wo, spo) & lt);
       }
-      __syncthreads();
-      const u32 sp_n = bn * 0x01010101u, sp_o = bo * 0x01010101u;
-      u32 c_on = 0, c_no = 0;
+      const i32 dn = (i32)(c_nn >> 3) - (i32)(c_on >> 3), dq = (i32)(c_no >> 3) - (i32)(c_oo >> 3);
+      fnb[h] = (u32)((i32)F[bn[h]] + dn);
+      fob[h] = (u32)((i32)F[bo[h]] + dq) + (bo[h] == bn[h]);
+    }
+    __syncwarp();
+    double2 a[2], b[2];
 #pragma unroll
-      for (int q = 0; q < 8; q++) {
-        c_on += __popc(__vcmpeq4(rowo[q], sp_n) & S.pm_lt[q][l]);
-        c_no += __popc(__vcmpeq4(rown[q], sp_o) & S.pm_le[q][l]);
+    for (int h = 0; h < 2; h++) {
+      if (valid[h]) { atomicAdd(&F[bn[h]], 1u); atomicSub(&F[bo[h]], 1u); }
+      a[h] = b[h] = make_double2(0.0, 0.0);
+      if (valid[h]) {
+        a[h] = make_double2(__ldg(&T[fnb[h]]), __ldg(&T[fnb[h] + 1]));
+        b[h] = make_double2(__ldg(&T[fob[h]]), __ldg(&T[fob[h] - 1]));
       }
-      c_on >>= 3; c_no >>= 3;
-      u32 fnb = 0, fob = 1;
-      if (valid) {
-        fnb = S.F[bn] + (S.Pn[w][bn] + c_nn) - (S.Po[w][bn] + c_on);
-        fob = S.F[bo] + (S.Pn[w][bo] + c_no) - (S.Po[w][bo] + c_oo);
-      }
-      const double c1 = T[fnb], c2 = T[fnb + 1], c3 = T[fob], c4 = T[fob - 1];
-      double mine = 0.0;
-      u32 start = 0;
-      double E = entropy;
-      int attempts = 0;
-      bool finished = false;
-      while (!finished) {
-        if (E >= 0x1p-12 && E < 8.0 && attempts < 12) {
-          const int eb = (int)((__double_as_longlong(E) >> 52) & 0x7FF) - 1023;
-          const double blo = pow2d(eb);
-          const bool one = (E - blo >= 0.75) && (2.0 * blo - E > 0.75);
-          const int B = one ? eb : ((E < 1.5 * blo) ? eb - 1 : eb);
-          const double scale = pow2d(52 - B), inv = pow2d(B - 52);
-          const bool part = valid && tid >= start;
-          if (tid == 0) S.firstbad = 0xFFFFFFFFu;
-          const double d[4] = {-c1, c2, -c3, c4};
-          i64s kb, k;
-          bool mybad;
-          if (one) seg_scan<2>(S, E, scale, pow2d(B + 1), part, d, kb, k, mybad);
-          else seg_scan<4>(S, E, scale, pow2d(B + 1), part, d, kb, k, mybad);
-          if (__syncthreads_or(mybad) == 0) {
-            if (part) mine = (double)k * inv;
-            if ((int)tid == steps - 1) S.entropy = mine;
-            finished = true;
-          } else {
-            if (mybad) atomicMin(&S.firstbad, tid);
-            __syncthreads();
-            const u32 fb = S.firstbad;
-            if (part && tid < fb) mine = (double)k * inv;
-            if (tid == fb) {
-              double ee = (double)kb * inv;
-              ee = __dsub_rn(ee, c1);
-              ee = __dadd_rn(ee, c2);
-              ee = __dsub_rn(ee, c3);
-              ee = __dadd_rn(ee, c4);
-              mine = ee;
-              S.restartE = ee;
-              if ((int)tid == steps - 1) S.entropy = ee;
-            }
-            __syncthreads();
-            E = S.restartE;
-            start = fb + 1;
-            attempts++;
-            if ((int)start >= steps) finished = true;
-          }
-        } else {
-          S.terms[tid * 4 + 0] = c1; S.terms[tid * 4 + 1] = c2; S.terms[tid * 4 + 2] = c3; S.terms[tid * 4 + 3] = c4;
-          __syncthreads();
-          if (w == 0) {
-            double e = E;
-            for (int k = (int)start; k < steps; k++) {
-              const double2 ab = *reinterpret_cast<const double2 *>(&S.terms[k * 4]);
-              const double2 cd = *reinterpret_cast<const double2 *>(&S.terms[k * 4 + 2]);
-              e = __dsub_rn(e, ab.x);
-              e = __dadd_rn(e, ab.y);
-              e = __dsub_rn(e, cd.x);
-              e = __dadd_rn(e, cd.y);
-              if (l == 0) S.series[k] = e;
-            }
-            if (l == 0) S.entropy = e;
-          }
-          __syncthreads();
-          if (tid >= start) mine = S.series[tid];
-          finished = true;
-        }
-      }
-      const i32 sp = i + 1 - SEG_WINDOW;
-      bool maybe[2];
+    }
+    if (l == 0) while (g + 1 - (i32)*vcons >= SG_SLOTS) __nanosleep(256);
+    __syncwarp();
 #pragma unroll
-      for (int p = 0; p < 2; p++) {
-        maybe[p] = act[p] && (i0 + steps - SEG_WINDOW - index_mark[p] > ithr[p]);
-        if (maybe[p] && valid && fabs(__dsub_rn(mine, mark[p])) > thr[p] && (sp - index_mark[p] > ithr[p])) atomicMin(&S.first[p], tid);
-      }
-      if (lead_n) S.Hn[w][bn] = 0;
-      if (lead_o) S.Ho[w][bo] = 0;
-      __syncthreads();
-      S.F[tid] = (u32)((i32)S.F[tid] + dF);
-#pragma unroll
-      for (int p = 0; p < 2; p++) if (maybe[p] && S.first[p] == tid) S.cutval[p] = mine;
-      __syncthreads();
-      entropy = S.entropy;
-#pragma unroll
-      for (int p = 0; p < 2; p++) {
-        if (maybe[p] && S.first[p] != 0xFFFFFFFFu) {
-          const i32 seg_point = i0 + (i32)S.first[p] + 1 - SEG_WINDOW;
-          if (tid == 0 && cnt[p] < B2_MAX_SEG - 1) out[p][cnt[p]] = (u32)seg_point;
-          cnt[p]++;
-          index_mark[p] = seg_point;
-          mark[p] = S.cutval[p];
-        }
-      }
-      __syncthreads();
+    for (int h = 0; h < 2; h++) {
+      ring[(g + h) % SG_SLOTS][l][0] = a[h];
+      ring[(g + h) % SG_SLOTS][l][1] = b[h];
     }
-  }
-  if (tid == 0) {
-    for (int k = 0; k < 2; k++) {
-      if (len > 0) { if (cnt[k] < B2_MAX_SEG) out[k][cnt[k]] = (u32)len; cnt[k]++; }
-    }
-    __threadfence();
-    nseg[2 * c] = cnt[0]; nseg[2 * c + 1] = cnt[1];
+    __syncwarp();
+    if (l == 0) { __threadfence_block(); *vprod = (u32)min(g + 2, ng); }
   }
 }
 
 int b2k_segment(cudaStream_t st, const u8 *d_in, const B2Chunk *d_chunks, u32 n_chunks, const double *d_T,
-                u32 *d_seg, u32 *d_nseg, const u32 *d_progress) {
+                u32 *d_seg, u32 *d_nseg) {
   if (n_chunks == 0) return 0;
-  k_segment<<<n_chunks, SG_THREADS, 0, st>>>(d_in, d_chunks, n_chunks, d_T, d_seg, d_nseg, d_progress);
+  k_segment<<<n_chunks, SG_THREADS, 0, st>>>(d_in, d_chunks, n_chunks, d_T, d_seg, d_nseg);
   B2_CUDA_CHECK(cudaGetLastError());
   return 0;
 }
```

Result: slower. 1791 (median of 6 runs) (-2.0%).
